# chenxy99/Scanpaths

Hardware: AMD Instinct MI355X
Metric: images/sec/GPU (AiR train step, bs=32, 320x512) at 1/2/4/8 MI355X (higher is better)
Workload: dtype f32; 1 GPU; AiR supervised train step (fwd+loss+bwd+clip+Adam), resnet50, T=16, 320x512, per-GPU batch 32; global_batch=32, parallelism=dp1

## Files before the change

include/scanpaths_amd.h:

```cpp
#ifndef SCANPATHS_AMD_H
#define SCANPATHS_AMD_H
#include <stdint.h>

#ifdef __cplusplus
extern "C" {
#endif

#define SP_OK 0
#define SP_EINVAL (-1)
#define SP_ENULL (-2)

#define SP_ABI_VERSION 4
int sp_abi_version(void);

int sp_set_tuning(const char* name, int value);
int sp_timing_build(void);

typedef struct sp_conv_desc {
    int N_img, Hi, Wi, Kc, ldx;
    int Ho, Wo, Nout, ldc;
    int KH, KW, stride, pad, dil;
    int mode, ldw;
    float alpha;
    int beta, relu;
    int nbatch;
    int64_t strideX, strideW, strideC;
    int ksplit;
    void* workspace;
    int w_scale_rows;
    const int* row_last;
    int row_step;
} sp_conv_desc;

int sp_conv_igemm(const sp_conv_desc* d, const float* X, const float* W, const float* bias, float* out, void* stream);

int sp_split3_bf16(const float* x, int64_t n, void* out, void* stream);
int sp_split3_bf16_wT(const float* w, int Co, int taps, int Ci, void* out, void* stream);
int sp_conv_igemm_bf16x3(const sp_conv_desc* d, const void* Xsplit, const void* Wsplit, const float* bias, float* out,
                         void* stream);

typedef struct sp_wgrad_desc {
    int N_img, Hi, Wi, Ci, ldx;
    int Ho, Wo, Co, ldy;
    int KH, KW, stride, pad, dil;
    int ldo;
    int beta;
    float alpha;
    int nbatch;
    int64_t strideX, strideY, strideO;
    int x_scale_vec, y_scale_vec;
    const int* row_last;
    int row_step;
} sp_wgrad_desc;

int64_t sp_conv_wgrad_workspace(const sp_wgrad_desc* d);
int sp_conv_wgrad(const sp_wgrad_desc* d, const float* X, const float* dY, float* dW, void* workspace, void* stream);

int64_t sp_conv_wgrad_bf16x3_workspace(const sp_wgrad_desc* d);
int sp_conv_wgrad_bf16x3(const sp_wgrad_desc* d, const void* Xsplit, const void* dYsplit, float* dW, void* workspace,
                         void* stream);

int sp_split2_f16(const float* x, int64_t n, void* out, float* scale_amax,
                  int have_amax ,
                  void* stream);
int sp_split2_f16_wT(const float* w, int Co, int taps, int Ci, void* out, float* scale_amax, void* stream);
int sp_split2_f16_rows(const float* w, int64_t rows, int64_t K, int Kc, const float* absorb, void* out, float* row_scale, void* stream);
int sp_split2_f16_wT_rows(const float* w, int nbatch, int Co, int taps, int Ci, const float* absorb, void* out, float* row_scale, void* stream);
int64_t sp_split2_f16_cols_workspace(int64_t rows, int C);
int sp_split2_f16_cols(const float* x, int64_t rows, int C, void* out, float* col_scale, void* scratch, void* stream);
int sp_conv_igemm_f16x2(const sp_conv_desc* d, const void* Xsplit, const float* x_scale, const void* Wsplit, const float* w_scale,
                        const float* bias, float* out, void* stream);
int64_t sp_conv_wgrad_f16x2_workspace(const sp_wgrad_desc* d);
int sp_conv_wgrad_f16x2(const sp_wgrad_desc* d, const void* Xsplit, const float* x_scale, const void* dYsplit,
                        const float* y_scale, float* dW, void* workspace, void* stream);
int64_t sp_conv_wgrad_f16x2_multi_workspace(const sp_wgrad_desc* d, int nseg);
int sp_conv_wgrad_f16x2_multi(const sp_wgrad_desc* d, int nseg, const void* const* Xsplits, const float* const* x_scales,
                              const void* const* dYsplits, const float* const* y_scales, float* dW, void* workspace,
                              const int* row_last, const int* seg_steps, void* stream);
int64_t sp_conv_stats_tiles(const sp_conv_desc* d);
int sp_conv_igemm_f16x2_stats(const sp_conv_desc* d, const void* Xsplit, const float* x_scale, const void* Wsplit,
                              const float* w_scale, float* out, double* st_partial, float* st_mm, void* stream);
int sp_conv_igemm_f16x1(const sp_conv_desc* d, const void* Xsplit, const float* x_scale, const void* Wsplit, const float* w_scale,
                        const float* bias, float* out, void* stream);
int sp_conv_wgrad_f16x1(const sp_wgrad_desc* d, const void* Xsplit, const float* x_scale, const void* dYsplit,
                        const float* y_scale, float* dW, void* workspace, void* stream);
int sp_gateconv_lstm_f16x2(const sp_conv_desc* d, const void* Hsplit, const float* h_scale, const void* Wsplit, const float* w_scale,
                           const float* xg, const float* c_prev, const float* spcol, const float* wc, int P, int KP, float* gates,
                           float* c_out, float* h_out, unsigned* h_amax,
                           void* hout_planes ,
                           float* hout_scale , float hout_bound ,
                           void* stream);
int sp_rank1_grads_applies(int B, int P, int N3, int KP, int ldy);
int64_t sp_rank1_grads_workspace(int B, int P, int N3, int KP);
int sp_rank1_grads_f16x2(const void* dpre_planes, const float* dpre_scale, int ldy, const void* wcT_planes, const float* wcT_row_scale,
                         const float* spcol, int B, int P, int N3, int KP, float* dsp, float* dwc, void* workspace, const int* row_last,
                         int row_step, void* stream);


int64_t sp_colsum_workspace(int64_t M, int C);
int sp_colsum(const float* x, int64_t M, int C, int ld, float* out, int beta, void* workspace, void* stream);
int sp_rowsum(const float* x, int64_t M, int C, float scale, float* out, void* stream);
int sp_rowsum_bwd(const float* dout, int64_t M, int C, float scale, float* dx, void* stream);

int64_t sp_bn_workspace(int64_t M, int C);
int sp_bn_stats(const float* x, int64_t M, int C, float eps, float momentum, float* mean, float* invstd,
                float* running_mean, float* running_var, void* workspace, void* stream);
int sp_bn_eval_stats(const float* running_mean, const float* running_var, int C, float eps, float* mean,
                     float* invstd, void* stream);
int sp_bn_apply(const float* x, const float* mean, const float* invstd, const float* gamma, const float* beta,
                const float* residual, int relu, int64_t M, int C, float* y,
                unsigned* y_amax , void* stream);
int sp_bn_backward(const float* dy, const float* x, const float* y, const float* mean, const float* invstd,
                   const float* gamma, int relu, int training, int64_t M, int C, float* dx, float* dres,
                   float* dgamma, float* dbeta, void* workspace,
                   unsigned* dx_amax , void* stream);

int64_t sp_bn_split_workspace(int64_t M, int C);
int64_t sp_bn_mask_words(int64_t M, int C);
int sp_bn_fwd_split(const float* x, int64_t M, int C, float eps, float momentum, const float* gamma, const float* beta,
                    const float* residual, const unsigned* res_amax, int relu, float* mean, float* invstd, float* running_mean,
                    float* running_var, float* ext, float* y, void* planes, float* y_scale, unsigned* bound,
                    unsigned long long* mask, void* workspace,
                    const double* pre_partial ,
                    const float* pre_mm , int pre_G, void* stream);
int sp_bn_bwd_split(const float* dy, const float* x, const unsigned long long* mask, const float* mean, const float* invstd,
                    const float* gamma, const float* ext, int64_t M, int C, float* dx, float* dres, void* planes, float* dx_scale,
                    unsigned* bound, float* dgamma, float* dbeta, void* workspace, void* stream);

int sp_maxpool3s2_fwd(const float* x, int N, int H, int W, int C, float* y, unsigned char* argmax , int Ho, int Wo,
                      void* stream);
int sp_maxpool3s2_bwd(const float* dy, const unsigned char* argmax, int N, int H, int W, int C, float* dx, int Ho, int Wo, void* stream);
int sp_nchw_to_nhwc_pad(const float* x, int N, int C, int H, int W, int Cp, float* y, void* stream);
int sp_pad_lastdim(const float* x, int64_t rows, int Cin, int Cout, float* y, void* stream);
int sp_sum_n(const float* const* inputs, int count, int64_t n, float* out, unsigned* out_amax, const int* row_last, const int* steps,
             int nsamples, void* stream);
int sp_sum_n_mixed(const float* const* inputs, const void* const* planes, const float* const* scales, int count, int64_t n, float* out,
                   unsigned* out_amax, const int* row_last, const int* steps, int nsamples, void* stream);
int sp_relu_bwd(const float* dy, const float* y, int64_t n, float* dx, void* stream);
int sp_add(const float* a, const float* b, float* out, int64_t n, void* stream);

int sp_lstm_pointwise_fwd(const float* xg, const float* hg, const float* c_prev, int64_t rows, int C, float* gates,
                          float* c_out, float* h_out, void* stream);
int sp_lstm_rank1_fwd(const float* xg, const float* hg, const float* c_prev, const float* spcol, const float* wc, int B, int P,
                      int C, int KP, float* gates, float* c_out, float* h_out,
                      unsigned* h_amax , void* stream);
int64_t sp_rank1_dwc_workspace(int B, int P, int N3, int KP);
int sp_rank1_dwc(const float* dpre, const float* spcol, int B, int P, int ld, int N3, int KP, void* workspace, float* dwc,
                 void* stream);
int64_t sp_sempool_workspace(int S, int B, int P, int C);
int sp_sempool_fwd(const float* a, const float* vf, int S, int B, int P, int C, float alpha, void* workspace, float* out, int sbc,
                   void* stream);
int sp_sempool_bwd(const float* dout, const float* out, const float* a, const float* vf, int S, int B, int P, int C, float alpha,
                   float* da, float* dvf, const int* row_last, int row_step, int sbc, void* stream);
int sp_lstm_pointwise_bwd(const float* dh, const float* dc, const float* gates, const float* c_prev, const float* c_out,
                          int64_t rows, int C, float* dpre, float* dc_prev, unsigned* dpre_amax, unsigned* dcp_amax,
                          const unsigned* dh_amax, const unsigned* dc_amax, float c_bound, float cprev_bound, void* planes,
                          float* dpre_scale, const int* row_last, int row_step, int rows_per_sample, void* stream);

int sp_im2col3x3_1ch(const float* maps, int S, int R, int H, int W, int ldk, float* col, void* stream);
int sp_col2im3x3_1ch(const float* dcol, int S, int R, int H, int W, int ldk, float* dmaps, void* stream);

int sp_listatt_fwd(const float* L, const float* u, int T, int R, int D, float* mem, float* alpha, void* stream);
int sp_listatt_bwd(const float* dmem, const float* L, const float* u, const float* alpha, int T, int R, int D, float* dL,
                   float* du_partial, void* stream);

int sp_mulrelu_fwd(const float* a, const float* b, int64_t n, int64_t nb, float* out, void* stream);
int sp_mulrelu_bwd(const float* dout, const float* a, const float* b, const float* out, int64_t n, int64_t nb, float* da,
                   float* db_partial, void* stream);

int sp_select_rows(const float* a, const float* b, const unsigned char* sel, int64_t rows, int64_t len, float* out,
                   void* stream);
int sp_select_rows_bwd(const float* dout, const unsigned char* sel, int64_t rows, int64_t len, float* da, float* db,
                       void* stream);

int sp_head_finish_fwd(const float* Z, int B, int Hm, int Wm, int ldz, int nheads, int HC, const float* cb,
                       int cb_per_sample , const float* w2, const float* b2, int softmax, float* logits, float* amap, float* mu,
                       float* sigma2, float* drt,
                       const float* dpre ,
                       int zc , int parts, void* stream);
int sp_head_finish_bwd(const float* dlogits, int64_t dlogits_ld, const float* damap , const float* dmu,
                       const float* dsigma2, const float* logits, const float* amap, const float* sigma2, const float* drt, int B, int Hm,
                       int Wm, int ldz, int nheads, int HC, const float* w2, int softmax, float* dZ, float* dcb_partial,
                       float* dw2_partial, float* db2_partial,
                       float* ddpre ,
                       int zc, int parts, int* live, void* stream);

int sp_head_num_classes(int Hm, int Wm);
int sp_head_compose11_fwd(const float* G, const float* cb, int nheads, int HC, int C, int Hm, int Wm, float* W11,
                          float* cbsum, void* stream);
int sp_head_compose11_bwd(const float* dW11, const float* dcbsum, int nheads, int HC, int C, int Hm, int Wm, float* dG,
                          float* dcb, void* stream);
int sp_sal_gather_fwd(const float* T, int B, int Hm, int Wm, int ldt, int nsel, const int* hmap, float* Z2, void* stream);
int sp_sal_gather_bwd(const float* dZ2, int B, int Hm, int Wm, int ldt, int nsel, int nsrc, const int* hmap, float* dT,
                      const int* row_last, int row_step, void* stream);
int sp_drt_direct_fwd(const float* h, const float* W11, const float* cbsum, const int* hmap, int B, int Hm, int Wm, int C,
                      int nsel, float* Dpre, void* stream);
int sp_drt_direct_bwd_data(const float* dDpre, const float* W11, const int* hmap, int B, int Hm, int Wm, int C, int nsel,
                           int accumulate, float* dh, const int* live, const int* row_last, int row_step, int rowB, void* stream);
int64_t sp_drt_direct_bwd_weight_workspace(int B, int Hm, int Wm, int C, int nsel);
int sp_drt_direct_bwd_weight(const float* dDpre, const float* h, const int* hmap, int B, int Hm, int Wm, int C, int nsel, int nheads,
                             void* workspace, float* dW11, float* dcbsum, const int* live, const int* row_last, int row_step, int rowB,
                             void* stream);

int sp_gemm_skinny_applies(int M, int N, int K, int lda, int ldb, int ldc, int layout);
int64_t sp_gemm_skinny_workspace(int M, int N, int K, int layout);
int sp_gemm_skinny(const float* A, const float* B, const float* bias, float* C, int M, int N, int K, int lda, int ldb, int ldc, int layout,
                   float alpha, int relu, void* workspace, void* stream);

int64_t sp_scanpath_loss_workspace(int B, int T);
int sp_scanpath_loss(const float* z, const float* gt, const float* amask, const float* mu, const float* sigma2,
// ... 105 lines not shown
```

scanpaths_amd/config.py:

```python
from __future__ import annotations

import os
import sys

DEFAULTS = {
    "split_scheme": "f16x2", "use_split": True, "library": "product", "always_reset_amax": False,
    "fused_amax": True, "grad_merge": True, "bn_split": True, "bn_skip_dx": True, "bn_skip_z": True, "lstm_bwd_split": True,
    "rank1_dsp_split": True, "rank1_dwc_split": True, "lstm_skip_dpre": True, "fuse_gate_lstm": True, "lstm_h_planes": True,
    "defer_wgrad": True, "channel_scales": True, "hw2_single": True, "row_sparsity": True, "direct_grad": True, "skinny_gemm": True, "async_dgrad": True,
    "drt_batched": True, "rank1_fused": True,
}
_off = lambda v: v != "0"
_ENV = {
    "SP_SPLIT_SCHEME": ("split_scheme", str), "SP_NO_SPLIT": ("use_split", lambda v: not v), "SP_LIBRARY": ("library", str),
    "SP_ALWAYS_RESET_AMAX": ("always_reset_amax", bool), "SP_NO_AMAX_HINT": ("fused_amax", lambda v: not v),
    "SP_GRAD_MERGE": ("grad_merge", _off), "SP_BN_SPLIT": ("bn_split", _off), "SP_BN_SKIP_DX": ("bn_skip_dx", _off),
    "SP_BN_SKIP_Z": ("bn_skip_z", _off), "SP_LSTM_BWD_SPLIT": ("lstm_bwd_split", _off), "SP_RANK1_DSP_SPLIT": ("rank1_dsp_split", _off),
    "SP_RANK1_DWC_SPLIT": ("rank1_dwc_split", _off), "SP_LSTM_SKIP_DPRE": ("lstm_skip_dpre", _off), "SP_FUSE_LSTM": ("fuse_gate_lstm", _off),
    "SP_LSTM_H_PLANES": ("lstm_h_planes", _off), "SP_DEFER_WGRAD": ("defer_wgrad", _off), "SP_CHANNEL_SCALES": ("channel_scales", _off),
    "SP_HW2_SINGLE": ("hw2_single", _off), "SP_ROW_SPARSITY": ("row_sparsity", _off), "SP_DIRECT_GRAD": ("direct_grad", _off), "SP_SKINNY_GEMM": ("skinny_gemm", _off),
    "SP_ASYNC_DGRAD": ("async_dgrad", _off), "SP_DRT_BATCHED": ("drt_batched", _off), "SP_RANK1_FUSED": ("rank1_fused", _off),
}
TIMING_KNOBS = {"SP_H2_DBG": b"h2_dbg", "SP_HW_DBG": b"hw_dbg", "SP_B3_DBG": b"b3_dbg", "SP_HW_SPLITS": b"hw_splits", "SP_H2_HALO": b"h2_halo",
                "SP_ROW_ORDER": b"row_order", "SP_HW_CAP": b"hw_cap"}

settings = dict(DEFAULTS)
_announced = set()


def env_tuning_allowed() -> bool:
    return os.environ.get("SP_ALLOW_ENV_TUNING") == "1"


def _loud(msg: str) -> None:
    if msg not in _announced:
        _announced.add(msg)
        print(f"scanpaths_amd.config: {msg}", file=sys.stderr, flush=True)


def _check(name, value):
    if name not in DEFAULTS:
        raise KeyError(f"scanpaths_amd.config: unknown switch {name!r} (known: {sorted(DEFAULTS)})")
    if name == "split_scheme" and value not in ("f16x2", "bf16x3", "f16x1"):
        raise ValueError(f"split_scheme must be f16x2, bf16x3 or f16x1, got {value!r}")
    if name == "library" and value not in ("product", "timing"):
        raise ValueError(f"library must be product or timing, got {value!r}")
    if name == "split_scheme" and value == "f16x1":
        _loud("THROUGHPUT MODE selected (split_scheme=f16x1): GEMM operands rounded to ONE fp16 plane -- about 100x off the 1e-4 parity "
              "bar; results are NOT comparable with the fp32 reference")
    if name == "library" and value == "timing":
        _loud("TIMING LIBRARY selected (libscanpaths_amd_timing.so): contains wrong-result timing modes; for tools/ only")


def _load_env():
    present = [k for k in list(_ENV) + list(TIMING_KNOBS) if os.environ.get(k) not in (None, "")]
    if not present:
        return
    if not env_tuning_allowed():
        _loud(f"IGNORING {', '.join(present)}: environment tuning needs SP_ALLOW_ENV_TUNING=1 (set switches in code with "
              "scanpaths_amd.config.set)")
        return
    for k in present:
        if k in _ENV:
            name, parse = _ENV[k]
            v = parse(os.environ[k])
            _check(name, v)
            settings[name] = v


def set(**kw) -> None:
    for k, v in kw.items():
        _check(k, v)
        if k == "library" and "scanpaths_amd.hip" in sys.modules and sys.modules["scanpaths_amd.hip"]._lib is not None \
                and v != settings["library"]:
            raise RuntimeError("scanpaths_amd.config: the library is already loaded; choose it before the first launch")
        settings[k] = v
    f = sys.modules.get("scanpaths_amd.functional")
    if f is not None:
        f._apply_config()
    h = sys.modules.get("scanpaths_amd.hip")
    if h is not None and "library" in kw:
        h._apply_config()


def honour_env_for_tools() -> None:
    os.environ["SP_ALLOW_ENV_TUNING"] = "1"
    _load_env()
    for name in ("scanpaths_amd.functional", "scanpaths_amd.hip"):
        m = sys.modules.get(name)
        if m is not None:
            if name.endswith("hip") and m._lib is not None and (settings["library"] == "timing") != m.TIMING_LIB:
                raise RuntimeError("scanpaths_amd.config: the library is already loaded; call honour_env_for_tools() before the first launch")
            m._apply_config()


def non_default() -> dict:
    return {k: v for k, v in settings.items() if v != DEFAULTS[k]}


_load_env()
# ... 1 lines not shown
```

scanpaths_amd/csrc/bn_pool.hip:

```cpp
#include "common.h"
#include <algorithm>

namespace {

__device__ __forceinline__ int64_t sp_cdiv_dev(int64_t a, int64_t b) { return (a + b - 1) / b; }

constexpr int CB = 64;
constexpr int RL = 16;
constexpr int MAX_G = 256;

inline int pick_G_wide(int64_t M, int C) {
    const int64_t colblocks = sp_cdiv(C, 256);
    int64_t g = sp_cdiv(1024, colblocks);
    g = std::min<int64_t>(g, sp_cdiv(M, 4 * 8));
    g = std::min<int64_t>(g, 1024);
    return (int)std::max<int64_t>(g, 1);
}

inline int pick_G(int64_t M, int C) {
    const int64_t colblocks = sp_cdiv(C, CB);
    int64_t g = sp_cdiv(2048, colblocks);
    g = std::min<int64_t>(g, sp_cdiv(M, RL * 8));
    g = std::min<int64_t>(g, MAX_G);
    return (int)std::max<int64_t>(g, 1);
// ... 852 lines not shown
extern "C" int sp_bn_apply(const float* x, const float* mean, const float* invstd, const float* gamma, const float* beta,
                           const float* residual, int relu, int64_t M, int C, float* y, unsigned* y_amax, void* stream) {
    if (!x || !mean || !invstd || !gamma || !beta || !y) return SP_ENULL;
    if (C % 4) return SP_EINVAL;
    const int64_t n4 = M * C / 4;
    SP_RESET_AMAX(y_amax, stream);
    hipLaunchKernelGGL(bn_apply_kernel, dim3(ew_blocks(n4)), dim3(256), 0, (hipStream_t)stream, x, mean, invstd, gamma,
                       beta, residual, relu, n4, C, y, y_amax);
    SP_LAUNCH_CHECK();
    return SP_OK;
}

extern "C" int sp_bn_backward(const float* dy, const float* x, const float* y, const float* mean, const float* invstd,
                              const float* gamma, int relu, int training, int64_t M, int C, float* dx, float* dres,
                              float* dgamma, float* dbeta, void* workspace, unsigned* dx_amax, void* stream) {
    if (!dy || !x || !mean || !invstd || !gamma || !dx || !dgamma || !dbeta || !workspace) return SP_ENULL;
    if (relu && !y) return SP_ENULL;
    if (C % 4 || M <= 0) return SP_EINVAL;
    hipStream_t s = (hipStream_t)stream;
    const int G = pick_G(M, C);
    double* partial = (double*)workspace;
    float* coef = (float*)(partial + (int64_t)G * 2 * C);
    hipLaunchKernelGGL(bn_bwd_partial, dim3((unsigned)sp_cdiv(C, CB), G), dim3(256), 0, s, dy, x, y, mean, invstd, relu, M,
                       C, G, partial);
    SP_LAUNCH_CHECK();
    hipLaunchKernelGGL(bn_bwd_final, dim3((unsigned)sp_cdiv(C, FIN_C)), dim3(FIN_C * FIN_L), 0, s, partial, M, C, G, dgamma, dbeta,
                       coef);
    SP_LAUNCH_CHECK();
    const int64_t n4 = M * C / 4;
    SP_RESET_AMAX(dx_amax, s);
    hipLaunchKernelGGL(bn_bwd_apply, dim3(ew_blocks(n4)), dim3(256), 0, s, dy, x, y, mean, invstd, gamma, coef, relu,
                       training, n4, C, dx, dres, dx_amax);
    SP_LAUNCH_CHECK();
    return SP_OK;
}

extern "C" int64_t sp_bn_split_workspace(int64_t M, int C) {
    const int64_t G = std::max(pick_G(M, C), pick_G_wide(M, C));
    return G * 2 * C * (int64_t)sizeof(double) + G * 2 * C * (int64_t)sizeof(float) + 2 * (int64_t)C * (int64_t)sizeof(float);
}

extern "C" int64_t sp_bn_mask_words(int64_t M, int C) { return sp_cdiv(M * C / 4, 64) * 4; }

extern "C" int sp_bn_fwd_split(const float* x, int64_t M, int C, float eps, float momentum, const float* gamma, const float* beta,
                               const float* residual, const unsigned* res_amax, int relu, float* mean, float* invstd,
                               float* running_mean, float* running_var, float* ext, float* y, void* planes, float* y_scale,
                               unsigned* bound, unsigned long long* mask, void* workspace, const double* pre_partial,
                               const float* pre_mm, int pre_G, void* stream) {
    if (!x || !gamma || !beta || !mean || !invstd || !ext || !y_scale || !bound || !workspace) return SP_ENULL;
    if ((residual && !res_amax) || (relu && !mask) || (!y && !planes)) return SP_ENULL;
    if (C % 4 || (planes && C % 16) || M <= 0 || ((uintptr_t)planes & 15)) return SP_EINVAL;
    hipStream_t s = (hipStream_t)stream;
    int G = pick_G(M, C);
    const double* partial = (double*)workspace;
    const float* mm = (float*)((double*)workspace + (int64_t)G * 2 * C);
    SP_RESET_AMAX(bound, s);
    if (pre_partial) {
        if (!pre_mm || pre_G < 1) return SP_EINVAL;
        partial = pre_partial;
        mm = pre_mm;
        G = pre_G;
    } else {
        hipLaunchKernelGGL(bn_stats_mm_partial, dim3((unsigned)sp_cdiv(C, CB), G), dim3(256), 0, s, x, M, C, G, (double*)workspace,
                           (float*)((double*)workspace + (int64_t)G * 2 * C));
        SP_LAUNCH_CHECK();
    }
    if (G > 256)
        hipLaunchKernelGGL((bn_stats_mm_final<8, 32>), dim3((unsigned)sp_cdiv(C, 8)), dim3(256), 0, s, partial, mm, M, C, G, eps,
                           momentum, gamma, beta, relu, mean, invstd, running_mean, running_var, ext, bound);
    else
        hipLaunchKernelGGL((bn_stats_mm_final<FIN_C, FIN_L>), dim3((unsigned)sp_cdiv(C, FIN_C)), dim3(256), 0, s, partial, mm, M, C,
                           G, eps, momentum, gamma, beta, relu, mean, invstd, running_mean, running_var, ext, bound);
    SP_LAUNCH_CHECK();
    const int64_t n4 = M * C / 4;
    hipLaunchKernelGGL(bn_apply_split_kernel, dim3(ew_blocks(n4)), dim3(256), 0, s, x, mean, invstd, gamma, beta, residual, bound,
                       residual ? res_amax : nullptr, relu, n4, C, y, (uint16_t*)planes, y_scale, relu ? mask : nullptr);
    SP_LAUNCH_CHECK();
    return SP_OK;
}

extern "C" int sp_bn_bwd_split(const float* dy, const float* x, const unsigned long long* mask, const float* mean,
                               const float* invstd, const float* gamma, const float* ext, int64_t M, int C, float* dx,
                               float* dres, void* planes, float* dx_scale, unsigned* bound, float* dgamma, float* dbeta,
                               void* workspace, void* stream) {
    if (!dy || !x || !mean || !invstd || !gamma || !ext || !dx_scale || !bound || !dgamma || !dbeta || !workspace) return SP_ENULL;
    if (!dx && !planes) return SP_ENULL;
    if (C % 4 || (planes && C % 16) || M <= 0 || ((uintptr_t)planes & 15)) return SP_EINVAL;
    hipStream_t s = (hipStream_t)stream;
    const bool wide = C >= 256 && C % 256 == 0;
    const int G = wide ? pick_G_wide(M, C) : pick_G(M, C);
    double* partial = (double*)workspace;
    float* dmax = (float*)(partial + (int64_t)G * 2 * C);
    float* coef = dmax + (int64_t)G * 2 * C;
    SP_RESET_AMAX(bound, s);
    if (wide)
        hipLaunchKernelGGL(bn_bwd_mm_partial<64>, dim3((unsigned)(C / 256), G), dim3(256), 0, s, dy, x, mask, mean, invstd, M, C, G,
                           partial, dmax);
    else
        hipLaunchKernelGGL(bn_bwd_mm_partial<16>, dim3((unsigned)sp_cdiv(C, CB), G), dim3(256), 0, s, dy, x, mask, mean, invstd, M, C,
                           G, partial, dmax);
    SP_LAUNCH_CHECK();
    if (G > 256)
        hipLaunchKernelGGL((bn_bwd_mm_final<8, 32>), dim3((unsigned)sp_cdiv(C, 8)), dim3(256), 0, s, partial, dmax, M, C, G, gamma,
                           mean, invstd, ext, dgamma, dbeta, coef, bound);
    else
        hipLaunchKernelGGL((bn_bwd_mm_final<FIN_C, FIN_L>), dim3((unsigned)sp_cdiv(C, FIN_C)), dim3(256), 0, s, partial, dmax, M, C,
                           G, gamma, mean, invstd, ext, dgamma, dbeta, coef, bound);
    SP_LAUNCH_CHECK();
    const int64_t n4 = M * C / 4;
    hipLaunchKernelGGL(bn_bwd_apply_split_kernel, dim3(ew_blocks(n4)), dim3(256), 0, s, dy, x, mask, mean, invstd, gamma, coef,
                       bound, n4, C, dx, dres, (uint16_t*)planes, dx_scale);
    SP_LAUNCH_CHECK();
    return SP_OK;
}

extern "C" int64_t sp_colsum_workspace(int64_t M, int C) { return (int64_t)pick_G(M, C) * C * (int64_t)sizeof(double); }

extern "C" int sp_colsum(const float* x, int64_t M, int C, int ld, float* out, int beta, void* workspace, void* stream) {
    if (!x || !out || !workspace) return SP_ENULL;
    if (C % 4 || ld % 4 || M <= 0) return SP_EINVAL;
    hipStream_t s = (hipStream_t)stream;
    if (M <= COLSUM_SMALL_M && ((uintptr_t)x & 15) == 0 && ((uintptr_t)out & 15) == 0) {
        hipLaunchKernelGGL(colsum_small_kernel, dim3((unsigned)sp_cdiv(C, 256)), dim3(64), 0, s, x, (int)M, C, ld, out, beta);
        SP_LAUNCH_CHECK();
        return SP_OK;
    }
    const int G = pick_G(M, C);
    hipLaunchKernelGGL(colsum_partial, dim3((unsigned)sp_cdiv(C, CB), G), dim3(256), 0, s, x, M, C, ld, G, (double*)workspace);
    SP_LAUNCH_CHECK();
    hipLaunchKernelGGL(colsum_final, dim3((unsigned)sp_cdiv(C, FIN_C)), dim3(FIN_C * FIN_L), 0, s, (const double*)workspace, C, G, out,
                       beta);
    SP_LAUNCH_CHECK();
    return SP_OK;
}

extern "C" int sp_rowsum(const float* x, int64_t M, int C, float scale, float* out, void* stream) {
    if (!x || !out) return SP_ENULL;
    if (C % 4) return SP_EINVAL;
    const int blocks = (int)std::max<int64_t>(1, std::min<int64_t>(sp_cdiv(M, 4), 4096));
    hipLaunchKernelGGL(rowsum_kernel, dim3(blocks), dim3(256), 0, (hipStream_t)stream, x, M, C, scale, out);
    SP_LAUNCH_CHECK();
    return SP_OK;
}

extern "C" int sp_rowsum_bwd(const float* dout, int64_t M, int C, float scale, float* dx, void* stream) {
    if (!dout || !dx) return SP_ENULL;
    if (C % 4) return SP_EINVAL;
    const int64_t n4 = M * C / 4;
    hipLaunchKernelGGL(rowsum_bwd_kernel, dim3(ew_blocks(n4)), dim3(256), 0, (hipStream_t)stream, dout, n4, C, scale, dx);
    SP_LAUNCH_CHECK();
    return SP_OK;
}

extern "C" int sp_maxpool3s2_fwd(const float* x, int N, int H, int W, int C, float* y, unsigned char* argmax, int Ho, int Wo,
                                 void* stream) {
    if (!x || !y) return SP_ENULL;
    if (C % 4) return SP_EINVAL;
    const int64_t total = (int64_t)N * Ho * Wo * (C / 4);
    hipLaunchKernelGGL(maxpool_fwd_kernel, dim3(ew_blocks(total)), dim3(256), 0, (hipStream_t)stream, x, N, H, W, C, y, Ho, Wo,
                       argmax);
    SP_LAUNCH_CHECK();
    return SP_OK;
}

extern "C" int sp_maxpool3s2_bwd(const float* dy, const unsigned char* argmax, int N, int H, int W, int C, float* dx, int Ho,
                                 int Wo, void* stream) {
    if (!dy || !argmax || !dx) return SP_ENULL;
    if (C % 4) return SP_EINVAL;
    const int64_t total = (int64_t)N * H * W * (C / 4);
    hipLaunchKernelGGL(maxpool_bwd_idx_kernel, dim3(ew_blocks(total) * 4), dim3(256), 0, (hipStream_t)stream, dy, argmax, N, H, W,
                       C, dx, Ho, Wo);
    SP_LAUNCH_CHECK();
    return SP_OK;
}

extern "C" int sp_nchw_to_nhwc_pad(const float* x, int N, int C, int H, int W, int Cp, float* y, void* stream) {
    if (!x || !y) return SP_ENULL;
    if (Cp < C) return SP_EINVAL;
    const int64_t total = (int64_t)N * H * W * Cp;
    hipLaunchKernelGGL(nchw_to_nhwc_pad_kernel, dim3(ew_blocks(total)), dim3(256), 0, (hipStream_t)stream, x, N, C, H, W, Cp, y);
    SP_LAUNCH_CHECK();
    return SP_OK;
}
// ... 76 lines not shown
```

scanpaths_amd/csrc/conv_f16x2.hip:

```cpp
#include "common.h"
#include <algorithm>
#include <cstdlib>

typedef _Float16 f16x8 __attribute__((ext_vector_type(8)));

namespace {

#define SP_GLDS16(src, dst)                                                                                      \
    __builtin_amdgcn_global_load_lds((const __attribute__((address_space(1))) void*)(src),                       \
                                     (__attribute__((address_space(3))) void*)(dst), 16, 0, 0)

constexpr int HBM = 256, HBN = 128, HBK = 32;
constexpr int HA_BYTES = HBM * 128;
constexpr int HB_BYTES = HBN * 128;
constexpr int HSTAGE = HA_BYTES + HB_BYTES;
constexpr int HNSTAGE = 3;
constexpr int HCHUNK_KT = 8;
constexpr int HALO_W = 64, HALO_ROWSLOTS = HALO_W + 2, HALO_NSLOT = 6 * HALO_ROWSLOTS;
constexpr int HALO_PIECES = (HALO_NSLOT + 7) / 8;
constexpr int HALO_A_BYTES = HALO_PIECES * 1024;
constexpr int HALO_LDS = 2 * HALO_A_BYTES + 3 * HB_BYTES;

struct H2Args {
    const uint16_t* X;
    const uint16_t* W;
    const float* bias;
    float* C;
    const float* sx;
    const float* sw;
    int sw_rows;
    int64_t M;
    int Hi, Wi, Kc;
    int ldx;
    int Ho, Wo, Nout, ldc;
    int KH, KW, stride, pad, dil;
    int64_t ldwb;
    int64_t w_bstride;
    int rows_per_batch;
    int ncblk, nkt, tiles_n;
    float alpha;
    int beta, relu;
    uint32_t x_bytes, w_bytes;
    const float* l_xg;
    const float* l_cprev;
    const float* l_spcol;
    const float* l_wc;
    float* l_gates;
    float* l_c;
    float* l_h;
    unsigned* l_hamax;
    uint16_t* l_hplanes;
    float* l_hscale;
    float l_hbound;
    int lC, lP, lKP;
    int l_probe;
    double* st_partial;
    float* st_mm;
    const int* row_last;
    int row_step;
    int row_nimg;
};

__device__ __forceinline__ float h2_sigmoid(float x) { return sp_sigmoid(x); }
__device__ __forceinline__ int halo_swz(int slot) { return ((slot >> 1) & 3) << 1; }

template <int MODE, int NPROD, bool CBM, bool LSTM = false, bool HALO = false, int DBG = 0>
__global__ __launch_bounds__(512, 2) void h2_kernel(H2Args p) {
    static_assert(!LSTM || MODE == 0, "the LSTM epilogue belongs to the forward build");
    static_assert(!HALO || (CBM && NPROD == 3 && DBG == 0), "the halo build extends the channel-block-major schedule only");
    extern __shared__ __attribute__((aligned(16))) unsigned char smem[];
    constexpr bool LSTM_T = LSTM;
    const int t = threadIdx.x;
    const int lane = t & 63;
    const int wave = __builtin_amdgcn_readfirstlane(t >> 6);
    const int wm = wave >> 1, wn = wave & 1;

#ifdef SP_TIMING_VARIANTS
    const int probe = p.l_probe;
    if ((probe >> 8) && blockIdx.x < 256) {
        const int G = (probe >> 8) & 15, step_us = 2 * ((probe >> 12) & 31);
        const long long wait = (long long)((blockIdx.x >> 3) % G) * step_us * 100;
        const long long t0 = __builtin_amdgcn_s_memrealtime();
        while ((long long)__builtin_amdgcn_s_memrealtime() - t0 < wait) __builtin_amdgcn_s_sleep(32);
    }
#else
    constexpr int probe = 0;
#endif
    const float sx_dev = p.sx[0], sw_dev = p.sw_rows ? 1.f : p.sw[0];
    int tn, tmi;
    bool mapped = false;
    if constexpr (MODE == 1 && !LSTM) {
        if (p.row_nimg > 0) {
            const int mine = lane < p.row_nimg ? p.row_last[lane] : -1;
            const uint64_t lm = __ballot(lane < p.row_nimg && mine >= p.row_step);
            const uint64_t all = p.row_nimg == 64 ? ~0ull : ((1ull << p.row_nimg) - 1ull);
            const int tps = (p.Ho * p.Wo) / HBM;
            const int nlive = __popcll(lm);
            const int nl = nlive * tps * p.tiles_n;
            const int bid = blockIdx.x;
            uint64_t mask;
            int tml;
            if (bid < nl) {
                supertile_map(xcd_remap(bid, nl), nlive * tps, p.tiles_n, tml, tn, CBM);
                mask = lm;
            } else {
                tn = (bid - nl) % p.tiles_n;
                tml = (bid - nl) / p.tiles_n;
                mask = all & ~lm;
            }
            for (int k = tml / tps; k > 0; --k) mask &= mask - 1ull;
            tmi = (__ffsll((unsigned long long)mask) - 1) * tps + tml % tps;
            mapped = true;
        }
    }
    if (!mapped) supertile_map(xcd_remap(blockIdx.x, gridDim.x), gridDim.x / p.tiles_n, p.tiles_n, tmi, tn, CBM);
    const int64_t m0 = (int64_t)tmi * HBM;
    const int n0 = LSTM ? tn * 32 : tn * HBN;
    if constexpr (!LSTM) {
        if (p.row_last != nullptr) {
            const int howo = MODE == 1 ? p.Ho * p.Wo : p.rows_per_batch;
            const int img = (int)(m0 / howo);
            if (howo % HBM == 0 && m0 < p.M && p.row_last[img] < p.row_step) {
                if (!p.beta) {
                    for (int i = t; i < HBM * (HBN / 4); i += 512) {
                        const int row = i / (HBN / 4), n = n0 + (i % (HBN / 4)) * 4;
                        const int64_t m = m0 + row;
                        if (m >= p.M) continue;
                        float* dst = p.C + m * p.ldc + n;
                        if ((p.ldc & 3) == 0 && n + 3 < p.Nout && (reinterpret_cast<uintptr_t>(p.C) & 15) == 0) {
                            *reinterpret_cast<float4*>(dst) = make_float4(0.f, 0.f, 0.f, 0.f);
                        } else {
                            for (int e = 0; e < 4; ++e)
                                if (n + e < p.Nout) dst[e] = 0.f;
                        }
                    }
                }
                return;
            }
        }
    }
    const int HoWo = p.Ho * p.Wo;

    int a_c8[4], a_py[4], a_px[4], a_boff[4];
    bool a_rowok[4];
// ... 562 lines not shown
            if (t == 0) {
                p.l_hscale[0] = hsc;
                p.l_hscale[1] = p.l_hbound;
            }
        }
        if (p.l_hamax) {
#pragma unroll
            for (int off = 32; off >= 1; off >>= 1) hmx = fmaxf(hmx, __shfl_xor(hmx, off));
            if (lane == 0 && hmx > 0.f) atomicMax(p.l_hamax, __float_as_uint(hmx));
        }
        return;
    }
    {
        const bool stats = MODE == 0 && p.st_partial != nullptr;
        const bool wide = (p.ldc & 3) == 0 && (p.Nout & 3) == 0 && (reinterpret_cast<uintptr_t>(p.C) & 15) == 0;
        float* stg = reinterpret_cast<float*>(smem) + wave * (64 * 68);
        const bool full_m = m0 + HBM <= p.M;
        double cs[4], cq[4];
        float cmn[4], cmx[4];
#pragma unroll
        for (int j = 0; j < 4; ++j) {
            const int n = n0 + wn * 64 + j * 16 + l16;
            const bool n_ok = n < p.Nout;
            const float bv = (n_ok && p.bias) ? p.bias[n] : 0.f;
            const float iswn = (p.sw_rows && n_ok) ? 1.f / ((!LSTM && !HALO) ? pre_sw[j] : p.sw[swrow0 + n]) : isw;
            cs[j] = 0.0;
            cq[j] = 0.0;
            cmn[j] = INFINITY;
            cmx[j] = -INFINITY;
            if (wide && full_m) {
                if (n_ok) {
                    if (stats) {
#pragma unroll
                        for (int i = 0; i < 4; ++i)
#pragma unroll
                            for (int r = 0; r < 4; ++r) {
                                const float v = p.alpha * (((tot4[i][j][r] + acc4[i][j][r]) * isx) * iswn) + bv;
                                stg[(i * 16 + 4 * g4 + r) * 68 + j * 16 + l16] = v;
                                cs[j] += (double)v;
                                cq[j] += (double)v * (double)v;
                                cmn[j] = fminf(cmn[j], v);
                                cmx[j] = fmaxf(cmx[j], v);
                            }
                    } else {
#pragma unroll
                        for (int i = 0; i < 4; ++i)
#pragma unroll
                            for (int r = 0; r < 4; ++r)
                                stg[(i * 16 + 4 * g4 + r) * 68 + j * 16 + l16] = p.alpha * (((tot4[i][j][r] + acc4[i][j][r]) * isx) * iswn) + bv;
                    }
                }
                continue;
            }
#pragma unroll
            for (int i = 0; i < 4; ++i)
#pragma unroll
                for (int r = 0; r < 4; ++r) {
                    const int row = i * 16 + 4 * g4 + r;
                    const int64_t m = m0 + wm * 64 + row;
                    float v = p.alpha * (((tot4[i][j][r] + acc4[i][j][r]) * isx) * iswn) + bv;
                    if (wide) {
                        stg[row * 68 + j * 16 + l16] = v;
                    } else if (n_ok && m < p.M) {
                        float* dst = p.C + m * p.ldc + n;
                        if (p.beta) v += *dst;
                        if (p.relu) v = fmaxf(v, 0.f);
                        *dst = v;
                    }
                    if (stats && n_ok && m < p.M) {
                        cs[j] += (double)v;
                        cq[j] += (double)v * (double)v;
                        cmn[j] = fminf(cmn[j], v);
                        cmx[j] = fmaxf(cmx[j], v);
                    }
                }
        }
        if (wide) {
            asm volatile("s_waitcnt lgkmcnt(0)" ::: "memory");
            const int cq4 = lane & 15, rsub = lane >> 4;
            const int n = n0 + wn * 64 + 4 * cq4;
            if (full_m && n0 + HBN <= p.Nout && !p.relu) {
                float* dst0 = p.C + (m0 + wm * 64 + rsub) * p.ldc + n;
                const float* src0 = stg + rsub * 68 + 4 * cq4;
                if (!p.beta) {
#pragma unroll
                    for (int ps = 0; ps < 16; ++ps)
                        *reinterpret_cast<float4*>(dst0 + (int64_t)(ps * 4) * p.ldc) = *reinterpret_cast<const float4*>(src0 + ps * 4 * 68);
                } else {
                    float4 o[16];
#pragma unroll
                    for (int ps = 0; ps < 16; ++ps) o[ps] = *reinterpret_cast<const float4*>(dst0 + (int64_t)(ps * 4) * p.ldc);
#pragma unroll
                    for (int ps = 0; ps < 16; ++ps) {
                        float4 v = *reinterpret_cast<const float4*>(src0 + ps * 4 * 68);
                        v.x += o[ps].x; v.y += o[ps].y; v.z += o[ps].z; v.w += o[ps].w;
                        *reinterpret_cast<float4*>(dst0 + (int64_t)(ps * 4) * p.ldc) = v;
                    }
                }
            } else
#pragma unroll
            for (int ps = 0; ps < 16; ++ps) {
                const int row = ps * 4 + rsub;
                const int64_t m = m0 + wm * 64 + row;
                if (m < p.M && n < p.Nout) {
                    float4 v = *reinterpret_cast<const float4*>(stg + row * 68 + 4 * cq4);
                    float4* dst = reinterpret_cast<float4*>(p.C + m * p.ldc + n);
                    if (p.beta) {
                        const float4 o = *dst;
                        v.x += o.x; v.y += o.y; v.z += o.z; v.w += o.w;
                    }
                    if (p.relu) {
                        v.x = fmaxf(v.x, 0.f); v.y = fmaxf(v.y, 0.f); v.z = fmaxf(v.z, 0.f); v.w = fmaxf(v.w, 0.f);
                    }
                    *dst = v;
                }
            }
        }
        if (stats) {
            asm volatile("s_waitcnt lgkmcnt(0)" ::: "memory");
            __builtin_amdgcn_s_barrier();
            double* sh_s = reinterpret_cast<double*>(smem);
            float* sh_m = reinterpret_cast<float*>(smem + 4 * HBN * 2 * sizeof(double));
#pragma unroll
            for (int j = 0; j < 4; ++j) {
#pragma unroll
                for (int off = 16; off <= 32; off <<= 1) {
                    cs[j] += __shfl_xor(cs[j], off);
                    cq[j] += __shfl_xor(cq[j], off);
                    cmn[j] = fminf(cmn[j], __shfl_xor(cmn[j], off));
                    cmx[j] = fmaxf(cmx[j], __shfl_xor(cmx[j], off));
                }
                if (g4 == 0) {
                    const int col = wn * 64 + j * 16 + l16;
                    sh_s[(wm * HBN + col) * 2 + 0] = cs[j];
                    sh_s[(wm * HBN + col) * 2 + 1] = cq[j];
                    sh_m[(wm * HBN + col) * 2 + 0] = cmn[j];
                    sh_m[(wm * HBN + col) * 2 + 1] = cmx[j];
                }
            }
            asm volatile("s_waitcnt lgkmcnt(0)" ::: "memory");
            __builtin_amdgcn_s_barrier();
            if (t < HBN && n0 + t < p.Nout) {
                double a = 0.0, b = 0.0;
                float mn = INFINITY, mx = -INFINITY;
#pragma unroll
                for (int w = 0; w < 4; ++w) {
                    a += sh_s[(w * HBN + t) * 2 + 0];
                    b += sh_s[(w * HBN + t) * 2 + 1];
                    mn = fminf(mn, sh_m[(w * HBN + t) * 2 + 0]);
                    mx = fmaxf(mx, sh_m[(w * HBN + t) * 2 + 1]);
                }
                const int64_t g = m0 / HBM;
                p.st_partial[(g * 2 + 0) * p.Nout + n0 + t] = a;
                p.st_partial[(g * 2 + 1) * p.Nout + n0 + t] = b;
                p.st_mm[(g * 2 + 0) * p.Nout + n0 + t] = mn;
                p.st_mm[(g * 2 + 1) * p.Nout + n0 + t] = mx;
            }
        }
    }
}

struct HWArgs {
    const uint16_t* X;
    const uint16_t* dY;
    float* out;
    const float* sx;
    const float* sy;
// ... 916 lines not shown
extern "C" int sp_split2_f16(const float* x, int64_t n, void* out, float* scale_amax, int have_amax, void* stream) {
    if (!x || !out || !scale_amax) return SP_ENULL;
    if (n % 16) return SP_EINVAL;
    hipStream_t s = (hipStream_t)stream;
    unsigned* amax = reinterpret_cast<unsigned*>(scale_amax + 1);
    if (!have_amax) {
        const int rc = launch_amax(x, n, amax, s);
        if (rc != SP_OK) return rc;
    }
    const int64_t n4 = n / 4;
    const int blocks = (int)std::max<int64_t>(1, std::min<int64_t>(sp_cdiv(n4, 256), 4096));
    hipLaunchKernelGGL(split2_kernel, dim3(blocks), dim3(256), 0, s, x, n4, amax, (uint16_t*)out, scale_amax);
    SP_LAUNCH_CHECK();
    return SP_OK;
}

extern "C" int sp_split2_f16_wT(const float* w, int Co, int taps, int Ci, void* out, float* scale_amax, void* stream) {
    if (!w || !out || !scale_amax) return SP_ENULL;
    if (((int64_t)taps * Co) % 16) return SP_EINVAL;
    hipStream_t s = (hipStream_t)stream;
    unsigned* amax = reinterpret_cast<unsigned*>(scale_amax + 1);
    const int64_t total = (int64_t)Co * taps * Ci;
    const int rc = launch_amax(w, total, amax, s);
    if (rc != SP_OK) return rc;
    const int blocks = (int)std::max<int64_t>(1, std::min<int64_t>(sp_cdiv(total, 256), 4096));
    hipLaunchKernelGGL(split2_wT_kernel, dim3(blocks), dim3(256), 0, s, w, Co, taps, Ci, amax, (uint16_t*)out, scale_amax);
    SP_LAUNCH_CHECK();
    return SP_OK;
}


extern "C" int sp_split2_f16_rows(const float* w, int64_t rows, int64_t K, int Kc, const float* absorb, void* out, float* row_scale,
                                  void* stream) {
    if (!w || !out || !row_scale) return SP_ENULL;
    if (rows < 1 || K < 16 || K % 16 || (absorb && (Kc < 4 || Kc % 4 || K % Kc))) return SP_EINVAL;
    if (rows > 0x7fffffff || (((uintptr_t)w | (uintptr_t)absorb) & 15)) return SP_EINVAL;
    hipLaunchKernelGGL(split2_rows_kernel, dim3((unsigned)rows), dim3(256), 0, (hipStream_t)stream, w, K, Kc, absorb, (uint16_t*)out,
                       row_scale, rows);
    SP_LAUNCH_CHECK();
    return SP_OK;
}

extern "C" int sp_split2_f16_wT_rows(const float* w, int nbatch, int Co, int taps, int Ci, const float* absorb, void* out,
                                     float* row_scale, void* stream) {
    if (!w || !out || !row_scale) return SP_ENULL;
    if (nbatch < 1 || nbatch > 65535 || ((int64_t)taps * Co) % 16 || Ci % 4 || Ci < 4 || ((uintptr_t)w & 15)) return SP_EINVAL;
    hipLaunchKernelGGL(split2_wT_rows_kernel, dim3(Ci / 4, nbatch), dim3(256), 0, (hipStream_t)stream, w, Co, taps, Ci, absorb, (uint16_t*)out,
                       row_scale);
    SP_LAUNCH_CHECK();
    return SP_OK;
}

static int colamax_blocks(int64_t rows, int C_) {
    const int C4 = C_ / 4, cg_per = std::min(C4, 256), rpb = 256 / cg_per;
    return (int)std::max<int64_t>(1, std::min<int64_t>(sp_cdiv(rows, (int64_t)rpb * 4), COLAMAX_MAXBLK));
}
extern "C" int64_t sp_split2_f16_cols_workspace(int64_t rows, int C_) {
    if (rows < 1 || C_ < 16 || C_ % 16) return 0;
    return (int64_t)colamax_blocks(rows, C_) * C_ * (int64_t)sizeof(float);
}
extern "C" int sp_split2_f16_cols(const float* x, int64_t rows, int C_, void* out, float* col_scale, void* scratch, void* stream) {
    if (!x || !out || !col_scale || !scratch) return SP_ENULL;
    if (rows < 1 || C_ < 16 || C_ % 16 || (((uintptr_t)x | (uintptr_t)col_scale | (uintptr_t)scratch) & 15)) return SP_EINVAL;
    hipStream_t s = (hipStream_t)stream;
    const int nblk = colamax_blocks(rows, C_);
    hipLaunchKernelGGL(colamax_partial_kernel, dim3(nblk), dim3(256), 0, s, x, rows, C_, (float*)scratch);
    SP_LAUNCH_CHECK();
    hipLaunchKernelGGL(colamax_final_kernel, dim3((unsigned)sp_cdiv(C_, 32)), dim3(256), 0, s, (const float*)scratch, nblk, C_, col_scale);
    SP_LAUNCH_CHECK();
    const int64_t n4 = rows * (C_ / 4);
    const int blocks2 = (int)std::max<int64_t>(1, std::min<int64_t>(sp_cdiv(n4, 256), 4096));
    hipLaunchKernelGGL(split2_cols_kernel, dim3(blocks2), dim3(256), 0, s, x, n4, C_, (const float*)col_scale, (uint16_t*)out);
    SP_LAUNCH_CHECK();
    return SP_OK;
}

static bool halo_applies(const sp_conv_desc* d) {
    return d->KH == 3 && d->KW == 3 && d->stride == 1 && d->dil == 1 && d->pad == 1 && d->Wo == HALO_W && d->Wi == HALO_W &&
           d->Hi == d->Ho && (d->Ho * d->Wo) % HBM == 0 && d->Kc % 32 == 0;
}

static int conv_igemm_f16(const sp_conv_desc* d, const void* Xs, const float* x_scale, const void* Ws, const float* w_scale,
                          const float* bias, float* out, void* stream, int nprod, double* st_partial = nullptr,
                          float* st_mm = nullptr) {
    if (!d || !Xs || !Ws || !x_scale || !w_scale || !out) return SP_ENULL;
    if (d->mode != 0 && d->mode != 1) return SP_EINVAL;
    if (d->Kc % 32 || d->ldx < d->Kc || d->ldx % 16) return SP_EINVAL;
    if (((uintptr_t)Xs | (uintptr_t)Ws) & 15) return SP_EINVAL;
    if (d->nbatch < 1 || d->stride < 1 || d->dil < 1) return SP_EINVAL;
    const int64_t rows_b = (int64_t)d->N_img * d->Ho * d->Wo;
    if (d->nbatch > 1) {
        if (d->mode != 0 || d->KH * d->KW != 1 || d->stride != 1 || d->pad != 0 || rows_b % HBM || rows_b >= (1LL << 31)) return SP_EINVAL;
        if (d->strideX != rows_b * d->ldx || d->strideC != rows_b * d->ldc || d->strideW != (int64_t)d->Nout * d->Kc) return SP_EINVAL;
        if (st_partial || nprod != 3) return SP_EINVAL;
    }
    H2Args a{};
    a.X = (const uint16_t*)Xs; a.W = (const uint16_t*)Ws; a.bias = bias; a.C = out;
    a.sx = x_scale; a.sw = w_scale; a.sw_rows = d->w_scale_rows ? 1 : 0;
    a.row_last = ((d->mode == 1 && d->nbatch == 1) || (d->mode == 0 && d->nbatch > 1)) ? d->row_last : nullptr; a.row_step = d->row_step;
    a.row_nimg = (a.row_last && d->mode == 1 && d->nbatch == 1 && d->N_img <= 64 && ((int64_t)d->Ho * d->Wo) % HBM == 0 &&
                  sp_tuning_get(SP_TUNE_ROW_ORDER, 1) == 1) ? d->N_img : 0;
    a.M = rows_b * d->nbatch;
    a.Hi = d->Hi; a.Wi = d->Wi; a.Kc = d->Kc; a.ldx = d->ldx;
    a.Ho = d->Ho; a.Wo = d->Wo; a.Nout = d->Nout; a.ldc = d->ldc;
    a.KH = d->KH; a.KW = d->KW; a.stride = d->stride; a.pad = d->pad; a.dil = d->dil;
    a.w_bstride = d->nbatch > 1 ? 4 * d->strideW : 0;
    a.rows_per_batch = (int)rows_b;
    a.ldwb = 4 * (int64_t)d->KH * d->KW * d->Kc;
    a.ncblk = d->Kc / 32;
    a.nkt = d->KH * d->KW * a.ncblk;
    a.tiles_n = (int)sp_cdiv(d->Nout, HBN);
    a.alpha = d->alpha; a.beta = d->beta; a.relu = d->relu;
    const int64_t xb = 4LL * d->nbatch * d->N_img * d->Hi * d->Wi * d->ldx, wb = 4LL * d->nbatch * d->Nout * d->KH * d->KW * d->Kc;
    if (xb + 64 >= (1LL << 32) || wb + 64 >= (1LL << 32)) return SP_EINVAL;
    a.x_bytes = (uint32_t)xb; a.w_bytes = (uint32_t)wb;
    if (a.M <= 0 || a.M >= (1LL << 31) || a.Nout <= 0) return SP_EINVAL;
    hipStream_t st = (hipStream_t)stream;
    const bool f = d->mode == 0;
    const bool cbm_ok = d->KH * d->KW > 1 && d->KH * d->KW <= 32 && (f || d->stride == 1);
    if (st_partial) {
        if (!f || !st_mm || nprod != 3 || d->beta || d->relu || bias) return SP_EINVAL;
        a.st_partial = st_partial; a.st_mm = st_mm;
        return cbm_ok ? launch_h2<0, 3, true>(a, st) : launch_h2<0, 3, false>(a, st);
    }
#ifdef SP_TIMING_VARIANTS
    if (sp_tuning_get(SP_TUNE_H2_DBG, 0) >= 256) a.l_probe = sp_tuning_get(SP_TUNE_H2_DBG, 0) & ~255;
    switch (sp_tuning_get(SP_TUNE_H2_DBG, 0)) {
        case 6: return f ? launch_h2<0, 3, false, false, false, 1>(a, st) : launch_h2<1, 3, false, false, false, 1>(a, st);
        case 7: return f ? launch_h2<0, 3, false, false, false, 2>(a, st) : launch_h2<1, 3, false, false, false, 2>(a, st);
        case 8: return f ? launch_h2<0, 3, false, false, false, 3>(a, st) : launch_h2<1, 3, false, false, false, 3>(a, st);
        case 9: return f ? launch_h2<0, 3, false, false, false, 9>(a, st) : launch_h2<1, 3, false, false, false, 9>(a, st);
        default: break;
    }
#endif
    if (nprod == 1)
        return f ? launch_h2<0, 1, false>(a, st) : launch_h2<1, 1, false>(a, st);
    if (cbm_ok && halo_applies(d) && sp_tuning_get(SP_TUNE_H2_HALO, 1) == 1)
        return f ? launch_h2<0, 3, true, false, true>(a, st) : launch_h2<1, 3, true, false, true>(a, st);
    if (cbm_ok) return f ? launch_h2<0, 3, true>(a, st) : launch_h2<1, 3, true>(a, st);
    return f ? launch_h2<0, 3, false>(a, st) : launch_h2<1, 3, false>(a, st);
}

extern "C" int sp_conv_igemm_f16x2(const sp_conv_desc* d, const void* Xs, const float* x_scale, const void* Ws,
                                   const float* w_scale, const float* bias, float* out, void* stream) {
    return conv_igemm_f16(d, Xs, x_scale, Ws, w_scale, bias, out, stream, 3);
}

extern "C" int64_t sp_conv_stats_tiles(const sp_conv_desc* d) {
    if (!d) return 0;
    return sp_cdiv((int64_t)d->N_img * d->Ho * d->Wo, HBM);
}
extern "C" int sp_conv_igemm_f16x2_stats(const sp_conv_desc* d, const void* Xs, const float* x_scale, const void* Ws,
                                         const float* w_scale, float* out, double* st_partial, float* st_mm, void* stream) {
    if (!st_partial || !st_mm) return SP_ENULL;
    return conv_igemm_f16(d, Xs, x_scale, Ws, w_scale, nullptr, out, stream, 3, st_partial, st_mm);
}

extern "C" int sp_conv_igemm_f16x1(const sp_conv_desc* d, const void* Xs, const float* x_scale, const void* Ws,
                                   const float* w_scale, const float* bias, float* out, void* stream) {
    return conv_igemm_f16(d, Xs, x_scale, Ws, w_scale, bias, out, stream, 1);
}

extern "C" int sp_gateconv_lstm_f16x2(const sp_conv_desc* d, const void* Hs, const float* h_scale, const void* Ws,
                                      const float* w_scale, const float* xg, const float* c_prev, const float* spcol,
                                      const float* wc, int P, int KP, float* gates, float* c_out, float* h_out, unsigned* h_amax,
                                      void* hout_planes, float* hout_scale, float hout_bound, void* stream) {
    if (!d || !Hs || !Ws || !h_scale || !w_scale || !xg || !spcol || !wc || !gates || !c_out || !h_out) return SP_ENULL;
    if (d->mode != 0 || d->Kc % 32 || d->ldx != d->Kc || d->nbatch != 1 || d->stride != 1 || d->dil < 1) return SP_EINVAL;
    if (d->Nout != 4 * d->Kc || d->Ho != d->Hi || d->Wo != d->Wi || d->KH * d->KW < 2 || d->KH * d->KW > 32) return SP_EINVAL;
    if (P != d->Ho * d->Wo || P % HBM || KP < 1 || KP > 32) return SP_EINVAL;
    if (((uintptr_t)Hs | (uintptr_t)Ws) & 15) return SP_EINVAL;
    if (((uintptr_t)xg | (uintptr_t)c_prev | (uintptr_t)gates | (uintptr_t)c_out | (uintptr_t)h_out) & 15) return SP_EINVAL;
    if (d->w_scale_rows && ((uintptr_t)w_scale & 15)) return SP_EINVAL;
    H2Args a{};
    a.X = (const uint16_t*)Hs; a.W = (const uint16_t*)Ws; a.bias = nullptr; a.C = nullptr;
    a.sx = h_scale; a.sw = w_scale; a.sw_rows = d->w_scale_rows ? 1 : 0;
    a.M = (int64_t)d->N_img * P;
    a.Hi = d->Hi; a.Wi = d->Wi; a.Kc = d->Kc; a.ldx = d->Kc;
    a.Ho = d->Ho; a.Wo = d->Wo; a.Nout = d->Nout; a.ldc = d->Nout;
    a.KH = d->KH; a.KW = d->KW; a.stride = 1; a.pad = d->pad; a.dil = d->dil;
    a.ldwb = 4 * (int64_t)d->KH * d->KW * d->Kc;
    a.ncblk = d->Kc / 32;
    a.nkt = d->KH * d->KW * a.ncblk;
    a.tiles_n = d->Kc / 32;
    a.alpha = 1.f; a.beta = 0; a.relu = 0;
    const int64_t xb = 4LL * a.M * d->Kc, wb = 4LL * d->Nout * d->KH * d->KW * d->Kc;
    if (xb + 64 >= (1LL << 32) || wb + 64 >= (1LL << 32) || a.M <= 0) return SP_EINVAL;
    a.x_bytes = (uint32_t)xb; a.w_bytes = (uint32_t)wb;
    a.l_xg = xg; a.l_cprev = c_prev; a.l_spcol = spcol; a.l_wc = wc;
    if (hout_planes && (!hout_scale || !(hout_bound > 0.f) || ((uintptr_t)hout_planes & 15))) return SP_EINVAL;
    a.l_gates = gates; a.l_c = c_out; a.l_h = h_out; a.l_hamax = h_amax;
    a.l_hplanes = (uint16_t*)hout_planes; a.l_hscale = hout_scale; a.l_hbound = hout_bound;
    a.lC = d->Kc; a.lP = P; a.lKP = KP;
    a.l_probe = sp_tuning_get(SP_TUNE_H2_DBG, 0);
    hipStream_t st = (hipStream_t)stream;
    SP_RESET_AMAX(h_amax, st);
    if (halo_applies(d) && sp_tuning_get(SP_TUNE_H2_HALO, 1) == 1) return launch_h2<0, 3, true, true, true>(a, st);
    return launch_h2<0, 3, true, true, false>(a, st);
}

extern "C" int64_t sp_conv_wgrad_f16x2_workspace(const sp_wgrad_desc* d) {
    if (!d) return 0;
    if (d->nbatch > 1) return 0;
    const int sp = hw_splits(d);
    return sp <= 1 ? 0 : (int64_t)sp * d->Co * d->ldo * (int64_t)sizeof(float);
}

static int launch_hw_reduce(const HWScales& sc, const float* slab, float* dW, int Co, int Ntot, int ldo, int splits, int64_t slab_stride,
                            float alpha, int beta, hipStream_t s) {
    const int64_t total = (int64_t)Co * Ntot;
    if (Ntot % 4 == 0 && ldo % 4 == 0 && slab_stride % 4 == 0 && sc.Ci % 4 == 0 && (((uintptr_t)slab | (uintptr_t)dW) & 15) == 0) {
        const int blocks = (int)std::min<int64_t>(sp_cdiv(total / 4, 256), 4096);
        hipLaunchKernelGGL(hw_reduce4_kernel, dim3(blocks), dim3(256), 0, s, slab, dW, Co, Ntot / 4, ldo / 4, splits, slab_stride / 4, alpha, sc, beta);
    } else {
        const int blocks = (int)std::min<int64_t>(sp_cdiv(total, 256), 4096);
        hipLaunchKernelGGL(hw_reduce_kernel, dim3(blocks), dim3(256), 0, s, slab, dW, Co, Ntot, ldo, splits, slab_stride, alpha, sc, beta);
    }
    SP_LAUNCH_CHECK();
    return SP_OK;
}

static int conv_wgrad_f16(const sp_wgrad_desc* d, const void* Xsplit, const float* x_scale, const void* dYsplit,
                          const float* y_scale, float* dW, void* workspace, void* stream, int nprod) {
    if (!d || !Xsplit || !dYsplit || !x_scale || !y_scale || !dW) return SP_ENULL;
    if (d->Ci % 16 || d->Co % 16 || d->ldx != d->Ci || d->ldy < d->Co || d->ldy % 16 || d->nbatch < 1) return SP_EINVAL;
    if (((uintptr_t)Xsplit | (uintptr_t)dYsplit) & 15) return SP_EINVAL;
    const int64_t rows_b = (int64_t)d->N_img * d->Ho * d->Wo;
    const bool batched = d->nbatch > 1;
    if (batched) {
        if (d->KH * d->KW != 1 || d->stride != 1 || d->pad != 0 || rows_b % 32 || nprod != 3) return SP_EINVAL;
        if (d->strideX != rows_b * d->Ci || d->strideY != rows_b * d->ldy || d->strideO != (int64_t)d->Co * d->ldo) return SP_EINVAL;
    } else if (d->ldo < d->KH * d->KW * d->Ci) {
        return SP_EINVAL;
    }
    HWArgs a;
    a.X = (const uint16_t*)Xsplit; a.dY = (const uint16_t*)dYsplit;
    a.sx = x_scale; a.sy = y_scale;
    a.sx_vec = d->x_scale_vec ? 1 : 0; a.sy_vec = d->y_scale_vec ? 1 : 0;
// ... 128 lines not shown
```

scanpaths_amd/functional.py:

```python
from __future__ import annotations

import ctypes as C
from collections import namedtuple
from typing import Optional

import torch
from torch.autograd import Function

from . import config as _config
from . import hip
from .hip import ConvDesc, WgradDesc, check, ptr


_KSPLIT_MIN_NKT, _KSPLIT_KT = 8, 4


def _timed(key_flops, launch):
    if hip.TIMER is None:
        return launch()
    return hip.TIMER.bracket(*key_flops(), launch)


def _gemm_desc(M, Nout, Kc, *, ldx, ldw, ldc, mode=0, alpha=1.0, beta=0, relu=0, nbatch=1, sX=0, sW=0, sC=0):
    return ConvDesc(N_img=M, Hi=1, Wi=1, Kc=Kc, ldx=ldx, Ho=1, Wo=1, Nout=Nout, ldc=ldc, KH=1, KW=1, stride=1, pad=0, dil=1, mode=mode,
                    ldw=ldw, alpha=float(alpha), beta=int(beta), relu=int(relu), nbatch=nbatch, strideX=sX, strideW=sW, strideC=sC)


def _gemm_wgrad_desc(M, Co, Ci, *, ldx, ldy, ldo, alpha=1.0, nbatch=1, sX=0, sY=0, sO=0):
    return WgradDesc(N_img=M, Hi=1, Wi=1, Ci=Ci, ldx=ldx, Ho=1, Wo=1, Co=Co, ldy=ldy, KH=1, KW=1, stride=1, pad=0, dil=1, ldo=ldo,
                     alpha=float(alpha), nbatch=nbatch, strideX=sX, strideY=sY, strideO=sO)


def _igemm(d: ConvDesc, X, W, bias, out):
    M_, Nout, Kc, mode, taps, nbatch = d.N_img * d.Ho * d.Wo, d.Nout, d.Kc, d.mode, d.KH * d.KW, d.nbatch
    aligned = all(t is None or t.data_ptr() % 16 == 0 for t in (X, W, out, bias))
    if (SKINNY_GEMM and taps == 1 and nbatch == 1 and M_ <= 64 and not d.beta and d.Hi == d.Ho and d.Wi == d.Wo and d.stride == 1
            and d.pad == 0 and aligned and d.ldc % 4 == 0 and hip.lib().sp_gemm_skinny_applies(M_, Nout, Kc, d.ldx, d.ldw, d.ldc, mode)):
        L = hip.lib()
        ws = hip.workspace(L.sp_gemm_skinny_workspace(M_, Nout, Kc, mode), X.device, slot=2)

        def launch_sk():
            check(L.sp_gemm_skinny(ptr(X), ptr(W), ptr(bias), ptr(out), M_, Nout, Kc, d.ldx, d.ldw, d.ldc, mode, d.alpha, d.relu,
                                   ptr(ws), hip.stream()), "sp_gemm_skinny")
        FUSION_COUNTS["skinny_gemm"] += 1
        return _timed(lambda: (("skinny_fwd" if mode == 0 else "skinny_dgrad", M_, Nout, Kc, "1x1", 1), 2.0 * M_ * Nout * Kc), launch_sk)
    if taps == 1 and nbatch == 1:
        tiles = ((M_ + 127) // 128) * ((Nout + 127) // 128)
        nkt = (Kc + 31) // 32
        if tiles <= 64 and nkt >= _KSPLIT_MIN_NKT:
            d.ksplit = max(2, min(nkt // _KSPLIT_KT, 512 // tiles))
            d.workspace = ptr(hip.workspace(d.ksplit * M_ * Nout * 4, X.device, slot=2))

    def launch():
        check(hip.lib().sp_conv_igemm(C.byref(d), ptr(X), ptr(W), ptr(bias), ptr(out), hip.stream()), "sp_conv_igemm")
    _timed(lambda: (("igemm_fwd" if mode == 0 else "igemm_dgrad", M_, Nout, taps * Kc, f"{d.KH}x{d.KW}", nbatch),
                    2.0 * M_ * Nout * taps * Kc * nbatch), launch)


def _wgrad(d: WgradDesc, X, dY, dW):
    L = hip.lib()
    ws = hip.workspace(L.sp_conv_wgrad_workspace(C.byref(d)), X.device, slot=0)
    def launch():
        check(L.sp_conv_wgrad(C.byref(d), ptr(X), ptr(dY), ptr(dW), ptr(ws), hip.stream()), "sp_conv_wgrad")
    _timed(lambda: (("wgrad", d.N_img * d.Ho * d.Wo, d.Co, d.KH * d.KW * d.Ci, f"{d.KH}x{d.KW}", d.nbatch),
                    2.0 * d.N_img * d.Ho * d.Wo * d.Co * d.KH * d.KW * d.Ci * d.nbatch), launch)


def _apply_config():
    g = globals()
    c = _config.settings
    g["FUSED_AMAX"] = bool(c["fused_amax"])
    g["USE_BF16X3"] = bool(c["use_split"])
    g["THROUGHPUT_MODE"] = c["split_scheme"] == "f16x1"
    g["SPLIT_SCHEME"] = "f16x2" if c["split_scheme"] == "f16x1" else c["split_scheme"]
    for name, key in (("GRAD_MERGE", "grad_merge"), ("BN_SPLIT", "bn_split"), ("BN_SKIP_DX", "bn_skip_dx"), ("BN_SKIP_Z", "bn_skip_z"),
                      ("LSTM_BWD_SPLIT", "lstm_bwd_split"), ("RANK1_DSP_SPLIT", "rank1_dsp_split"), ("RANK1_DWC_SPLIT", "rank1_dwc_split"),
                      ("LSTM_SKIP_DPRE", "lstm_skip_dpre"), ("FUSE_GATE_LSTM", "fuse_gate_lstm"), ("LSTM_H_PLANES", "lstm_h_planes"),
                      ("DEFER_WGRAD", "defer_wgrad"), ("CHANNEL_SCALES", "channel_scales"), ("HW2_SINGLE", "hw2_single"),
                      ("ROW_SPARSITY", "row_sparsity"), ("DIRECT_GRAD", "direct_grad"), ("SKINNY_GEMM", "skinny_gemm"), ("ASYNC_DGRAD", "async_dgrad"),
                      ("DRT_BATCHED", "drt_batched"), ("RANK1_FUSED", "rank1_fused")):
        g[name] = bool(c[key])


_apply_config()


FUSION_COUNTS = {"lstm_bwd_split": 0, "bn_bwd_split_operand": 0, "gateconv_lstm": 0, "gateconv_lstm_hplanes": 0,
                 "bn_fwd_split": 0, "bn_fwd_split_operand": 0, "bn_skip_z": 0, "bn_bwd_split": 0, "bn_skip_dx": 0,
                 "conv_bn_stats": 0, "grad_merge": 0, "rank1_dsp_split": 0, "rank1_dwc_split": 0, "lstm_skip_dpre": 0, "wgrad_multi": 0,
                 "row_sparse_bwd": 0, "fan_in_rows": 0, "direct_grad": 0, "output_gate": 0, "skinny_gemm": 0, "async_dgrad": 0,
                 "drt_fwd_batched": 0, "rank1_fused": 0}


def _grad_slot(param):
    if not DIRECT_GRAD or param is None or not getattr(param, "is_leaf", False) or not param.requires_grad:
        return None
    if getattr(param, "_sp_flat", None) is None:
        return None
    if getattr(param, "_backward_hooks", None):
        return None
    try:
        return param, torch.autograd.graph.get_gradient_edge(param).node
    except Exception:
        return None


def _take_grad_view(pn, phys_perm=None):
    if pn is None:
        return None, None
    param, node = pn
    try:
        if not torch._C._will_engine_execute_node(node):
            return None, None
    except RuntimeError:
        return None, None
    slot = param._sp_flat
    g = slot.peek(param)
    if g is None:
        return None, None
    v = g.permute(*phys_perm) if phys_perm is not None else g
    if not v.is_contiguous():
        return None, None
    slot.take()
    FUSION_COUNTS["direct_grad"] += 1
    return slot, v


class RowsCtx:
    __slots__ = ("last", "B")

    def __init__(self, last):
        self.last, self.B = last, int(last.numel())


class DecodeRows:
    __slots__ = ("rc",)

    def __init__(self):
        self.rc = None

    def at(self, t: int) -> "DecodeStep":
        return DecodeStep(t, self)


class DecodeStep(int):
    def __new__(cls, t, rows):
        o = int.__new__(cls, t)
        o.rows = rows
        return o


def rows_ctx(step, nsamples):
    tok = getattr(step, "rows", None)
    if tok is None or not ROW_SPARSITY:
        return None
    rc = tok.rc
    if rc is None or rc.B != nsamples:
        return None
    return rc


class _OutputGate(Function):
    @staticmethod
    def forward(ctx, tok, *outs):
        ctx.tok = tok
        ctx.set_materialize_grads(False)
        return tuple(o.view_as(o) for o in outs)

    @staticmethod
    def backward(ctx, *grads):
        tok = ctx.tok
        tok.rc = None
        live = [g for g in grads if g is not None]
        if ROW_SPARSITY and live:
# ... 122 lines not shown
        n = xc.numel()
        out = torch.empty(2 * n + 32, dtype=torch.float16, device=x.device)
        Cc = xc.shape[-1]
        if channel and CHANNEL_SCALES and hint is None and xc.dim() >= 2 and Cc % 16 == 0 and not THROUGHPUT_MODE:
            cscale = torch.empty(Cc, dtype=torch.float32, device=x.device)
            L = hip.lib()
            ws = hip.workspace(L.sp_split2_f16_cols_workspace(n // Cc, Cc), x.device, slot=1)
            check(L.sp_split2_f16_cols(ptr(xc), n // Cc, Cc, ptr(out), ptr(cscale), ptr(ws), hip.stream()), "sp_split2_f16_cols")
            op = SplitOperand(out, cscale, scheme, "cols")
        else:
            scale = hint if hint is not None else _scale_slot(x.device)
            check(hip.lib().sp_split2_f16(ptr(xc), n, ptr(out), ptr(scale), int(hint is not None), hip.stream()), "sp_split2_f16")
            op = SplitOperand(out, scale, scheme)
    if cache is not None:
        cache[scheme] = op
    return op


def _absorb_of(act: Optional[SplitOperand]) -> Optional[torch.Tensor]:
    return act.scale if (act is not None and act.kind == "cols") else None


def split_w(w2d: torch.Tensor, scheme: str, Kc: Optional[int] = None, absorb: Optional[torch.Tensor] = None) -> SplitOperand:
    if scheme == "bf16x3":
        return SplitOperand(split3(w2d), None, scheme)
    w2d = w2d.contiguous()
    K = w2d.shape[-1]
    rows = w2d.numel() // K
    out = torch.empty(2 * w2d.numel() + 32, dtype=torch.float16, device=w2d.device)
    rscale = torch.empty(rows, dtype=torch.float32, device=w2d.device)
    check(hip.lib().sp_split2_f16_rows(ptr(w2d), rows, K, Kc if Kc is not None else K, ptr(absorb), ptr(out), ptr(rscale), hip.stream()),
          "sp_split2_f16_rows")
    return SplitOperand(out, rscale, scheme, "rows", absorb)


def split_op_wT(wp: torch.Tensor, scheme: Optional[str] = None, absorb: Optional[torch.Tensor] = None) -> SplitOperand:
    Co, KH, KW, Ci = wp.shape
    scheme = scheme or _scheme_for(Co)
    if scheme == "bf16x3":
        return SplitOperand(split3_wT(wp), None, scheme)
    out = torch.empty(2 * wp.numel() + 32, dtype=torch.float16, device=wp.device)
    if Ci % 4 == 0:
        rscale = torch.empty(Ci, dtype=torch.float32, device=wp.device)
        check(hip.lib().sp_split2_f16_wT_rows(ptr(wp), 1, Co, KH * KW, Ci, ptr(absorb), ptr(out), ptr(rscale), hip.stream()),
              "sp_split2_f16_wT_rows")
        return SplitOperand(out, rscale, scheme, "rows", absorb)
    assert absorb is None
    scale = _scale_slot(wp.device)
    check(hip.lib().sp_split2_f16_wT(ptr(wp), Co, KH * KW, Ci, ptr(out), ptr(scale), hip.stream()), "sp_split2_f16_wT")
    return SplitOperand(out, scale, scheme)


def _weight_operand(wp, act: SplitOperand, wcache, transposed=False) -> SplitOperand:
    absorb = _absorb_of(act)
    key = ("wT" if transposed else "w", act.scheme)
    if absorb is None and wcache is not None and key in wcache:
        return wcache[key]
    if transposed:
        op = split_op_wT(wp, act.scheme, absorb)
    else:
        Co, KH, KW, Ci = wp.shape
        op = split_w(wp.reshape(Co, KH * KW * Ci), act.scheme, Ci, absorb)
    if absorb is None and wcache is not None:
        wcache[key] = op
    return op


COST_M_SCALE = 1.0


def _b3_pays(M, N, K, Kc, nbatch=1, a_elems=None, free_a=False):
    if not USE_BF16X3 or nbatch != 1 or Kc % 16 or N < 64:
        return False
    f16 = _scheme_for(Kc) == "f16x2"
    Mc = M * COST_M_SCALE
    flops = 2.0 * Mc * N * K
    split_bytes = (12.0 if f16 else 10.0) * ((0 if free_a else Mc * Kc) + N * K)
    bpe = 4.0 if f16 else 6.0
    if bpe * (a_elems if a_elems is not None else 4.0 * M * Kc) + 64 >= 2 ** 32 or bpe * N * K + 64 >= 2 ** 32:
        return False
    return flops * (1 / 1.1e14 - 1 / (4.0e14 if f16 else 2.5e14)) > split_bytes / 4e12 and flops > (1e9 if free_a else 2e9)


def _igemm_b3(d: ConvDesc, Xs, Ws, bias, out, stats=None, rows=None):
    assert Xs.scheme == Ws.scheme, (Xs.scheme, Ws.scheme)
    f16 = Xs.scheme == "f16x2"
    xscale = Xs.scale
    mode = d.mode
    if f16 and rows is not None and mode == 1:
        d.row_last, d.row_step = rows[0].last.data_ptr(), int(rows[1])
    if f16:
        d.w_scale_rows = int(Ws.kind == "rows")
        if Xs.kind == "cols":
            if Ws.absorbed is not Xs.scale:
                raise RuntimeError("scanpaths_amd: a per-channel-scaled operand met a weight operand that did not absorb its scales")
            xscale = _one(out.device)
        elif Ws.absorbed is not None:
            raise RuntimeError("scanpaths_amd: a weight operand that absorbed per-channel scales met another activation operand")

    def launch():
        if stats is not None:
            check(hip.lib().sp_conv_igemm_f16x2_stats(C.byref(d), ptr(Xs.buf), ptr(xscale), ptr(Ws.buf), ptr(Ws.scale), ptr(out),
                                                      ptr(stats[0]), ptr(stats[1]), hip.stream()), "sp_conv_igemm_f16x2_stats")
        elif f16:
            fn = hip.lib().sp_conv_igemm_f16x1 if THROUGHPUT_MODE else hip.lib().sp_conv_igemm_f16x2
            check(fn(C.byref(d), ptr(Xs.buf), ptr(xscale), ptr(Ws.buf), ptr(Ws.scale), ptr(bias), ptr(out), hip.stream()),
                  "sp_conv_igemm_f16x2")
        else:
            check(hip.lib().sp_conv_igemm_bf16x3(C.byref(d), ptr(Xs.buf), ptr(Ws.buf), ptr(bias), ptr(out), hip.stream()),
                  "sp_conv_igemm_bf16x3")

    def key_flops():
        M = d.N_img * d.Ho * d.Wo
        K = d.KH * d.KW * d.Kc
        pre = ("h1" if THROUGHPUT_MODE else "h2") if f16 else "b3"
        sparse = f16 and rows is not None and mode == 1
        return (pre + ("_fwd" if mode == 0 else "_dgrad") + ("_rows" if sparse else ""), M, d.Nout, K, f"{d.KH}x{d.KW}", 1), 2.0 * M * d.Nout * K
    _timed(key_flops, launch)


def _wgrad_scheme(Ci, Co) -> str:
    return "f16x2" if _scheme_for(Ci) == "f16x2" and _scheme_for(Co) == "f16x2" else "bf16x3"


def _w3_pays(M, Co, K, Ci, nbatch=1, free_splits=False):
    f16 = _wgrad_scheme(Ci, Co) == "f16x2"
    if not USE_BF16X3 or nbatch != 1 or Co % 16 or Co < 64 or (Ci % 128 and not f16):
        return False
    flops = 2.0 * M * COST_M_SCALE * Co * K
    split_bytes = 0.0 if free_splits else (12.0 if f16 else 10.0) * M * COST_M_SCALE * (Ci + Co)
    if 6.0 * M * max(Ci, Co) * 4 >= 2 ** 32:
        return False
    return flops * (1 / 1.0e14 - 1 / (3.2e14 if f16 else 1.6e14)) > split_bytes / 4e12 and flops > 2e9


HW2_SINGLE_MIN_FLOPS = 9e10


def _wgrad_b3(d: WgradDesc, Xs, dYs, dW):
    assert Xs.scheme == dYs.scheme, (Xs.scheme, dYs.scheme)
    L = hip.lib()
    f16 = Xs.scheme == "f16x2"
    if f16:
        d.x_scale_vec, d.y_scale_vec = int(Xs.kind == "cols"), int(dYs.kind == "cols")
    M, Co, K = d.N_img * d.Ho * d.Wo, d.Co, d.KH * d.KW * d.Ci
    big = L.sp_conv_wgrad_f16x2_multi_workspace(C.byref(d), 1) if (f16 and HW2_SINGLE and not THROUGHPUT_MODE
                                                                   and 2.0 * M * COST_M_SCALE * Co * K >= HW2_SINGLE_MIN_FLOPS) else 0
    ws = hip.workspace(big if big > 0 else (L.sp_conv_wgrad_f16x2_workspace if f16 else L.sp_conv_wgrad_bf16x3_workspace)(C.byref(d)),
                       dW.device, slot=0)

    def launch():
        if big > 0:
            FUSION_COUNTS["wgrad_multi"] += 1
            one = lambda t: (C.c_void_p * 1)(t.data_ptr())
            check(L.sp_conv_wgrad_f16x2_multi(C.byref(d), 1, one(Xs.buf), one(Xs.scale), one(dYs.buf), one(dYs.scale), ptr(dW), ptr(ws),
                                              None, None, hip.stream()), "sp_conv_wgrad_f16x2_multi")
        elif f16:
            fn = L.sp_conv_wgrad_f16x1 if THROUGHPUT_MODE else L.sp_conv_wgrad_f16x2
            check(fn(C.byref(d), ptr(Xs.buf), ptr(Xs.scale), ptr(dYs.buf), ptr(dYs.scale), ptr(dW), ptr(ws), hip.stream()),
                  "sp_conv_wgrad_f16x2")
        else:
            check(L.sp_conv_wgrad_bf16x3(C.byref(d), ptr(Xs.buf), ptr(dYs.buf), ptr(dW), ptr(ws), hip.stream()),
                  "sp_conv_wgrad_bf16x3")
    _timed(lambda: (((("h1" if THROUGHPUT_MODE else "h2") if f16 else "b3") + ("_wgrad_multi" if big > 0 else "_wgrad"), M, Co, K, f"{d.KH}x{d.KW}", 1),
                    2.0 * M * Co * K), launch)


class ConvGeom(namedtuple("ConvGeom", "N H W Ci Co KH KW stride pad dil Ho Wo")):
    __slots__ = ()

    @classmethod
    def of(cls, x_shape, Co, KH, KW, stride=1, pad=0, dil=1) -> "ConvGeom":
        N, H, W, Ci = x_shape
        return cls(N, H, W, Ci, Co, KH, KW, stride, pad, dil,
                   (H + 2 * pad - dil * (KH - 1) - 1) // stride + 1, (W + 2 * pad - dil * (KW - 1) - 1) // stride + 1)

    @property
    def M(self) -> int:
        return self.N * self.Ho * self.Wo

    @property
    def K(self) -> int:
        return self.KH * self.KW * self.Ci

    def fwd_desc(self, **kw) -> ConvDesc:
        return ConvDesc(N_img=self.N, Hi=self.H, Wi=self.W, Kc=self.Ci, ldx=self.Ci, Ho=self.Ho, Wo=self.Wo, Nout=self.Co, ldc=self.Co,
                        KH=self.KH, KW=self.KW, stride=self.stride, pad=self.pad, dil=self.dil, mode=0, ldw=self.K, alpha=1.0, nbatch=1, **kw)

    def dgrad_desc(self, split: bool, **kw) -> ConvDesc:
        return ConvDesc(N_img=self.N, Hi=self.Ho, Wi=self.Wo, Kc=self.Co, ldx=self.Co, Ho=self.H, Wo=self.W, Nout=self.Ci, ldc=self.Ci,
                        KH=self.KH, KW=self.KW, stride=self.stride, pad=self.pad, dil=self.dil, mode=1,
                        ldw=self.KH * self.KW * self.Co if split else self.Ci, alpha=1.0, nbatch=1, **kw)

    def wgrad_desc(self, **kw) -> WgradDesc:
        return WgradDesc(N_img=self.N, Hi=self.H, Wi=self.W, Ci=self.Ci, ldx=self.Ci, Ho=self.Ho, Wo=self.Wo, Co=self.Co, ldy=self.Co,
                         KH=self.KH, KW=self.KW, stride=self.stride, pad=self.pad, dil=self.dil, ldo=self.K, alpha=1.0, nbatch=1, **kw)

    def fwd_split(self, free_a=False, a_elems=None) -> bool:
        return _b3_pays(self.M, self.Co, self.K, self.Ci, a_elems=a_elems, free_a=free_a)

    def dgrad_split(self, free_a=False, a_elems=None) -> bool:
        return _b3_pays(self.N * self.H * self.W, self.Ci, self.KH * self.KW * self.Co, self.Co, a_elems=a_elems, free_a=free_a)

    @property
    def wgrad_scheme(self) -> str:
        return _wgrad_scheme(self.Ci, self.Co)

    def wgrad_split(self, free_splits=False) -> Optional[str]:
        return self.wgrad_scheme if _w3_pays(self.M, self.Co, self.K, self.Ci, free_splits=free_splits) else None


def _conv_fwd(g: ConvGeom, x, wp, bias, y, *, relu=False, wcache=None, channel=False, free_a=False, a_elems=None, bn_stats=False):
    d = g.fwd_desc(relu=int(relu))
    if not g.fwd_split(free_a, a_elems):
        _igemm(d, x, wp, bias, y)
        return None, None
    xs = split_op(x, channel=channel)
    wsplit = _weight_operand(wp, xs, wcache)
    stats = None
    if bn_stats and BN_SPLIT and xs.scheme == "f16x2" and not THROUGHPUT_MODE and bias is None and not relu:
        G = hip.lib().sp_conv_stats_tiles(C.byref(d))
        stats = (torch.empty((G, 2, g.Co), dtype=torch.float64, device=x.device),
                 torch.empty((G, 2, g.Co), dtype=torch.float32, device=x.device), G)
    _igemm_b3(d, xs, wsplit, bias, y, stats=stats)
    return xs, stats


def _conv_dgrad(g: ConvGeom, dy, wp, dx, *, dys=None, wcache=None, channel=False, free_a=False, a_elems=None, beta=0, rows=None):
    if not g.dgrad_split(free_a, a_elems):
        _fp32_required(dy, "the fp32 data-gradient GEMM")
        _igemm(g.dgrad_desc(False, beta=beta), dy, wp, None, dx)
        return None
    if dys is None or dys.scheme != _scheme_for(g.Co):
        dys = split_op(dy, channel=channel)
    _igemm_b3(g.dgrad_desc(True, beta=beta), dys, _weight_operand(wp, dys, wcache, transposed=True), None, dx, rows=rows)
    return dys


def _conv_wgrad(g: ConvGeom, x, dy, dwp, *, xs=None, dys=None, channel=False):
    wsch = g.wgrad_scheme
    dy_cached = getattr(dy, "_sp_cache", None)
    if dys is None and dy_cached is not None and wsch in dy_cached:
        dys = dy_cached[wsch]
    if dys is not None and dys.scheme != wsch:
        dys = None
    if g.wgrad_split(free_splits=xs is not None and dys is not None):
        _wgrad_b3(g.wgrad_desc(), xs if xs is not None else split_op(x, wsch, channel=channel),
                  dys if dys is not None else split_op(dy, wsch, channel=channel), dwp)
    else:
        _fp32_required(dy, "the fp32 weight-gradient GEMM")
        _wgrad(g.wgrad_desc(), x, dy, dwp)


def colsum(x2d: torch.Tensor, C_: int, ld: int, M: int) -> torch.Tensor:
    out = torch.empty(C_, dtype=torch.float32, device=x2d.device)
    L = hip.lib()
    ws = hip.workspace(L.sp_colsum_workspace(M, C_), x2d.device, slot=1)
    check(L.sp_colsum(ptr(x2d), M, C_, ld, ptr(out), 0, ptr(ws), hip.stream()), "sp_colsum")
    return out


def _colsum_any(x: torch.Tensor, C_: int) -> torch.Tensor:
    M = x.numel() // C_
    if C_ % 4 == 0:
        return colsum(x, C_, C_, M)
    Cp = (C_ + 3) // 4 * 4
    xp = torch.empty((M, Cp), dtype=torch.float32, device=x.device)
    check(hip.lib().sp_pad_lastdim(ptr(x), M, C_, Cp, ptr(xp), hip.stream()), "sp_pad_lastdim")
    return colsum(xp, Cp, Cp, M)[:C_]


def _add_raw(a: torch.Tensor, b: torch.Tensor) -> torch.Tensor:
    a, b = a.contiguous(), b.contiguous()
    out = torch.empty_like(a)
    check(hip.lib().sp_add(ptr(a), ptr(b), ptr(out), a.numel(), hip.stream()), "sp_add")
    return out


class _Add(Function):
    @staticmethod
    def forward(ctx, a, b):
        return _add_raw(a, b)

    @staticmethod
    def backward(ctx, g):
        return g, g


class _ZeroGradTouch(Function):
    @staticmethod
    def forward(ctx, t, *params):
        ctx.shapes = [(p.shape, p.stride(), p.device) for p in params]
        return t.view_as(t)

    @staticmethod
    def backward(ctx, g):
        zeros = tuple(torch.zeros(sh, dtype=torch.float32, device=dev) for sh, _, dev in ctx.shapes)
        return (g,) + zeros


def touch_zero_grad(t, params):
    return _ZeroGradTouch.apply(t, *params)


class _FanOut(Function):
    @staticmethod
    def forward(ctx, x, n, token, step=None, events=None):
        ctx.n, ctx.token, ctx.step, ctx.events = n, token, step, events
        ctx.set_materialize_grads(False)
        return tuple(x.view_as(x) for _ in range(n))

    @staticmethod
    def backward(ctx, *grads):
        if ctx.events:
            cur = torch.cuda.current_stream()
            for ev in ctx.events.values():
                cur.wait_event(ev)
            ctx.events.clear()
# ... 2 lines not shown
            if grads[i] is None:
                raise RuntimeError(f"scanpaths_amd: fan-out alias {i} recorded a split-only gradient but no gradient arrived for it")
        idx = [i for i, g in enumerate(grads) if g is not None]
        if not idx:
            return None, None, None, None, None
        for i in idx:
            if i not in tok and getattr(grads[i], "_sp_skipped", False):
                raise RuntimeError("scanpaths_amd: a gradient whose fp32 form was left unwritten reached a fan-in without its record")
        gs = [grads[i].contiguous() for i in idx]
        ops = [tok.get(i) for i in idx]
        tok.clear()
        if any(op is not None for op in ops):
            out = torch.empty_like(gs[0])
            n = out.numel()
            assert n % 16 == 0 and len(gs) <= 32, (n, len(gs))
            f = (C.c_void_p * len(gs))(*[None if op is not None else g.data_ptr() for g, op in zip(gs, ops)])
            pl = (C.c_void_p * len(gs))(*[op.buf.data_ptr() if op is not None else None for op in ops])
            sc = (C.c_void_p * len(gs))(*[op.scale.data_ptr() if op is not None else None for op in ops])
            hint = _amax_hint(out.device)
            rcs = [op.rows[0] for op in ops if op is not None and op.rows is not None]
            rc = rcs[0] if (rcs and all(r is rcs[0] for r in rcs) and (n // rcs[0].B) % 16 == 0 and n % rcs[0].B == 0) else None
            steps = (C.c_int * len(gs))(*[(op.rows[1] if (op is not None and op.rows is not None) else -1) for op in ops]) if rc else None
            check(hip.lib().sp_sum_n_mixed(f, pl, sc, len(gs), n, ptr(out), _hint_ptr(hint), ptr(rc.last) if rc else None, steps,
                                           rc.B if rc else 0, hip.stream()), "sp_sum_n_mixed")
            if hint is not None:
                out._sp_amax = hint
            return out, None, None, None, None
        if len(gs) == 1:
            return gs[0], None, None, None, None
        out = torch.empty_like(gs[0])
        n = out.numel()
        if n % 4 or len(gs) > 32:
            acc = gs[0]
            for g in gs[1:]:
                acc = _add_raw(acc, g)
            return acc, None, None, None, None
        arr = (C.c_void_p * len(gs))(*[g.data_ptr() for g in gs])
        hint = _amax_hint(out.device)
        rc0 = rows_ctx(ctx.step, gs[0].shape[0]) if gs[0].dim() > 1 else None
        marks = [getattr(grads[i], "_sp_rows", None) for i in idx]
        if rc0 is None and any(m is not None for m in marks):
            cand = next(m[0] for m in marks if m is not None)
            if gs[0].dim() > 1 and cand.B == gs[0].shape[0] and ROW_SPARSITY:
                rc0 = cand
        steps = None
        if rc0 is not None and n % rc0.B == 0 and (n // rc0.B) % 4 == 0:
            if ctx.step is not None:
                steps = [int(ctx.step)] * len(gs)
            else:
                steps = [int(m[1]) if (m is not None and m[0] is rc0) else -1 for m in marks]
        sparse = steps is not None and any(st >= 0 for st in steps)
        if sparse:
            FUSION_COUNTS["fan_in_rows"] += 1
        check(hip.lib().sp_sum_n(arr, len(gs), n, ptr(out), _hint_ptr(hint), ptr(rc0.last) if sparse else None,
                                 (C.c_int * len(gs))(*steps) if sparse else None, rc0.B if sparse else 0, hip.stream()), "sp_sum_n")
        if hint is not None:
            out._sp_amax = hint
        return out, None, None, None, None


def fanout(x: torch.Tensor, n: int, step=None):
    split_ok = x.numel() % 16 == 0 and n <= 32
    token = {} if split_ok else None
    events = {} if (ASYNC_DGRAD and step is not None and x.is_cuda) else None
    outs = _FanOut.apply(x, n, token, step, events)
    if events is not None:
        for i, o in enumerate(outs):
            o._sp_fan_ev = (events, i)
    for attr in ("_sp_cache", "_sp_amax"):
        v = getattr(x, attr, None)
        if v is not None:
            for o in outs:
                setattr(o, attr, v)
    if split_ok:
        for i, o in enumerate(outs):
            o._sp_fan = (token, i)
            o._sp_split_grad_ok = True
    return outs




class GradMerge:
    __slots__ = ("first", "merged")

    def __init__(self):
        self.first, self.merged = None, False


class _Tap(Function):
    @staticmethod
    def forward(ctx, x, holder):
        ctx.holder = holder
        return x.view_as(x), x.view_as(x)

    @staticmethod
    def backward(ctx, g_main, g_side):
        h = ctx.holder
        merged, h.first, h.merged = h.merged, None, False
        if g_main is None or g_side is None:
            return (g_main if g_side is None else g_side), None
        if merged:
            return g_main, None
        return _add_raw(g_main.contiguous(), g_side.contiguous()), None


def tap(x: torch.Tensor, holder: GradMerge):
    outs = _Tap.apply(x, holder)
    for attr in ("_sp_cache", "_sp_amax"):
        v = getattr(x, attr, None)
        if v is not None:
            for o in outs:
                setattr(o, attr, v)
    return outs


class _ScaleConst(Function):
    @staticmethod
    def forward(ctx, x, c):
        x = x.contiguous()
        ctx.c = float(c)
        cs = torch.full((1,), float(c), dtype=torch.float32, device=x.device)
        out = torch.empty_like(x)
        check(hip.lib().sp_scale_by(ptr(x), ptr(cs), x.numel(), ptr(out), hip.stream()), "sp_scale_by")
        return out

    @staticmethod
    def backward(ctx, g):
        return _ScaleConst.apply(g, ctx.c), None


def scale_const(x: torch.Tensor, c: float) -> torch.Tensor:
    return _ScaleConst.apply(x, c)


def add(a: torch.Tensor, b: torch.Tensor) -> torch.Tensor:
    return _Add.apply(a, b)


def _phys(w: torch.Tensor) -> torch.Tensor:
    p = w.permute(0, 2, 3, 1)
    return p if p.is_contiguous() else p.contiguous()


class _Conv2d(Function):
    @staticmethod
    def forward(ctx, x, w, bias, stride, pad, dil, relu, wcache=None, bn_stats=False, grad_store=None, grad_accum=None, step=None):
        ctx.grad_store, ctx.grad_accum, ctx.step = grad_store, grad_accum, step
        ctx.w_param = _grad_slot(w) if w.dim() == 4 else None
        defer = wcache.get("defer") if isinstance(wcache, dict) else None
        ctx.defer_final = defer.claim() if (defer is not None and ctx.needs_input_grad[1]) else False
        ctx.dy_token = None
        x = x.contiguous()
        wp = _phys(w.detach())
        assert wp.shape[3] == x.shape[3], (wp.shape, x.shape)
        need_dx, need_dw = ctx.needs_input_grad[:2]
        g = ConvGeom.of(x.shape, *wp.shape[:3], stride, pad, dil)
        y = torch.empty((g.N, g.Ho, g.Wo, g.Co), dtype=torch.float32, device=x.device)
        shared = getattr(x, "_sp_cache", None) is not None
        if getattr(x, "_sp_uninit", False) and not conv_runs_from_split(x.shape, w, stride, pad, dil, need_dw):
            raise RuntimeError("scanpaths_amd: a BatchNorm left this input's fp32 form unwritten (skip_z) but this conv does not run "
                               "from the split operand alone; run with SP_BN_SKIP_DX=0")
        xs, stats = _conv_fwd(g, x, wp, bias, y, relu=relu, wcache=wcache, channel=True, free_a=shared, a_elems=x.numel(), bn_stats=bn_stats)
        if xs is not None:
            y._sp_from_split = xs.scheme == "f16x2"
            if stats is not None:
                FUSION_COUNTS["conv_bn_stats"] += 1
                y._sp_bnstats = stats
            keep = need_dw and g.wgrad_split(free_splits=True) == xs.scheme
            if (y._sp_from_split and g.wgrad_scheme == "f16x2" and bias is None and not relu and (not need_dw or keep)
                    and (not need_dx or g.dgrad_split(free_a=True, a_elems=y.numel()))):
                ctx.dy_token = y._sp_dy_token = {"skipped": False}
            if not keep:
                xs = None
        ctx.xs_scheme = (xs.scheme, xs.kind) if xs is not None else None
        xs_buf, xs_scale = (xs.buf, xs.scale) if xs is not None else (None, None)
        ctx.geom, ctx.cfg = g, (relu, bias is not None)
        ctx.wcache = wcache
        ctx.save_for_backward(x, wp, y if relu else None, xs_buf, xs_scale)
        return y

    @staticmethod
    def backward(ctx, dy):
        relu, has_bias = ctx.cfg
        x, wp, y, xs_buf, xs_scale = ctx.saved_tensors
        xs = SplitOperand(xs_buf, xs_scale, *ctx.xs_scheme) if xs_buf is not None else None
        if ctx.dy_token is not None and ctx.dy_token["skipped"] and getattr(dy, "_sp_cache", None) is None:
            raise RuntimeError("scanpaths_amd: a BatchNorm left this gradient's fp32 form unwritten (skip_dx) but its split form "
                               "did not arrive with it; run with SP_BN_SKIP_DX=0")
        dy = dy.contiguous()
        if relu:
            dyr = torch.empty_like(dy)
            check(hip.lib().sp_relu_bwd(ptr(dy), ptr(y), dy.numel(), ptr(dyr), hip.stream()), "sp_relu_bwd")
            dy = dyr
        dx, dw = _conv_backward(ctx.geom, x, wp, dy, xs, ctx.wcache, ctx.needs_input_grad[0], ctx.needs_input_grad[1],
                                accum=ctx.grad_accum, defer_final=ctx.defer_final, step=ctx.step, w_param=ctx.w_param)
        if ctx.grad_store is not None and dx is not None:
            ctx.grad_store.first = dx
        db = _colsum_any(dy, wp.shape[0]) if (has_bias and ctx.needs_input_grad[2]) else None
        return dx, dw, db, None, None, None, None, None, None, None, None, None




class DeferredWgrad:
    __slots__ = ("items", "claimed")

    def __init__(self):
        self.items, self.claimed = [], False

    def claim(self) -> bool:
        first, self.claimed = not self.claimed, True
        return first


def _flush_deferred(defer, wp, g: ConvGeom):
    items, defer.items, defer.claimed = defer.items, [], False
    if all(st is not None for _, _, st in items):
        items = sorted(items, key=lambda it: it[2])
    dwp = torch.empty_like(wp)
    L = hip.lib()
    xs0, dys0, _ = items[0]
    same = all(x.kind == xs0.kind and y.kind == dys0.kind for x, y, _ in items)
    steps = [st for _, _, st in items]
    toks = [getattr(st, "rows", None) for st in steps]
    rc = rows_ctx(steps[0], g.N) if (toks and toks[0] is not None and all(tk is toks[0] for tk in toks)) else None
    d = g.wgrad_desc(x_scale_vec=int(xs0.kind == "cols"), y_scale_vec=int(dys0.kind == "cols"))
    nseg = len(items)
    wsb = L.sp_conv_wgrad_f16x2_multi_workspace(C.byref(d), nseg) if (same and not THROUGHPUT_MODE and 1 < nseg <= 16) else 0
    if wsb > 0:
        ws = hip.workspace(wsb, wp.device, slot=3)
        arr = lambda ts: (C.c_void_p * nseg)(*[t.data_ptr() for t in ts])
        Xa, Sxa = arr([x.buf for x, _, _ in items]), arr([x.scale for x, _, _ in items])
        Ya, Sya = arr([y.buf for _, y, _ in items]), arr([y.scale for _, y, _ in items])
        seg_steps = (C.c_int * nseg)(*steps) if rc is not None else None
        if rc is not None:
            FUSION_COUNTS["row_sparse_bwd"] += 1

        def launch():
            check(L.sp_conv_wgrad_f16x2_multi(C.byref(d), nseg, Xa, Sxa, Ya, Sya, ptr(dwp), ptr(ws), ptr(rc.last) if rc is not None else None,
                                              seg_steps, hip.stream()), "sp_conv_wgrad_f16x2_multi")
        FUSION_COUNTS["wgrad_multi"] += 1
        _timed(lambda: (("h2_wgrad_multi" + ("_rows" if rc is not None else ""), g.M * nseg, g.Co, g.K, f"{g.KH}x{g.KW}", nseg),
                        2.0 * g.M * nseg * g.Co * g.K), launch)
    else:
        for k, (x, y, _) in enumerate(items):
            _wgrad_b3(g.wgrad_desc(beta=int(k > 0)), x, y, dwp)
    return dwp.permute(0, 3, 1, 2)


def _conv_backward(g: ConvGeom, x, wp, dy, xs, wcache, need_dx, need_dw, accum=None, defer_final=False, step=None, w_param=None):
    dx = dw = None
    dys = None
    dy_cached = getattr(dy, "_sp_cache", None)
    defer = wcache.get("defer") if (DEFER_WGRAD and isinstance(wcache, dict)) else None
    rc = rows_ctx(step, g.N)
    deferred = False
    if need_dw and defer is not None:
        wsch = g.wgrad_scheme
        have = dy_cached is not None and wsch in dy_cached
        if wsch == "f16x2" and xs is not None and xs.scheme == wsch and g.wgrad_split(free_splits=have):
            dys = dy_cached[wsch] if have else split_op(dy, wsch, channel=True)
            defer.items.append((xs, dys, step))
            deferred = True
    if need_dx:
        beta = 0
        if accum is not None and accum.first is not None and accum.first.shape == x.shape and accum.first.is_contiguous():
            dx, beta, accum.merged = accum.first, 1, True
            FUSION_COUNTS["grad_merge"] += 1
        else:
            dx = torch.empty_like(x)
        dys = _conv_dgrad(g, dy, wp, dx, dys=dys, wcache=wcache, channel=True, free_a=dy_cached is not None or dys is not None,
                          a_elems=dy.numel(), beta=beta, rows=(rc, step) if rc is not None else None) or dys
    slot = None
    if need_dw and not deferred:
        if defer is None:
            slot, dwp = _take_grad_view(w_param, (0, 2, 3, 1))
        if slot is None:
            dwp = torch.empty_like(wp)
        _conv_wgrad(g, x, dy, dwp, xs=xs, dys=dys, channel=True)
        if slot is not None:
            slot.done()
        else:
            dw = dwp.permute(0, 3, 1, 2)
    if need_dw and defer is not None and defer_final and defer.items:
        dsum = _flush_deferred(defer, wp, g)
        dw = dsum if dw is None else dw + dsum
    return dx, dw


def _geom_of_logical(x_shape, w, stride=1, pad=0, dil=1) -> ConvGeom:
    return ConvGeom.of(x_shape, w.shape[0], w.shape[2], w.shape[3], stride, pad, dil)


def conv_takes_split(x_shape, w, stride=1, pad=0, dil=1) -> bool:
    g = _geom_of_logical(x_shape, w, stride, pad, dil)
    return _scheme_for(g.Ci) == "f16x2" and g.fwd_split(free_a=True, a_elems=g.N * g.H * g.W * g.Ci)


def conv_runs_from_split(x_shape, w, stride=1, pad=0, dil=1, need_dw=True) -> bool:
    if not conv_takes_split(x_shape, w, stride, pad, dil):
        return False
    return (not need_dw) or _geom_of_logical(x_shape, w, stride, pad, dil).wgrad_split(free_splits=True) == "f16x2"


def conv2d(x, w, bias=None, stride=1, pad=0, dil=1, relu=False, wcache=None, bn_stats=False, grad_store=None, grad_accum=None, step=None):
    return _Conv2d.apply(x, w, bias, stride, pad, dil, relu, wcache, bn_stats, grad_store, grad_accum, step)


class _PadLast(Function):
    @staticmethod
    def forward(ctx, x, cout):
        x = x.contiguous()
        cin = x.shape[-1]
        rows = x.numel() // cin
        y = torch.empty(x.shape[:-1] + (cout,), dtype=torch.float32, device=x.device)
        check(hip.lib().sp_pad_lastdim(ptr(x), rows, cin, cout, ptr(y), hip.stream()), "sp_pad_lastdim")
        ctx.cin = cin
        return y

    @staticmethod
    def backward(ctx, dy):
        dy = dy.contiguous()
        cout = dy.shape[-1]
        rows = dy.numel() // cout
        dx = torch.empty(dy.shape[:-1] + (ctx.cin,), dtype=torch.float32, device=dy.device)
        check(hip.lib().sp_pad_lastdim(ptr(dy), rows, cout, ctx.cin, ptr(dx), hip.stream()), "sp_pad_lastdim")
        return dx, None


def pad_last(x, cout):
    return _PadLast.apply(x, cout)


def nchw_to_nhwc(x: torch.Tensor, cpad: int) -> torch.Tensor:
    x = x.contiguous()
    N, Cc, H, W_ = x.shape
    y = torch.empty((N, H, W_, cpad), dtype=torch.float32, device=x.device)
    check(hip.lib().sp_nchw_to_nhwc_pad(ptr(x), N, Cc, H, W_, cpad, ptr(y), hip.stream()), "sp_nchw_to_nhwc_pad")
    return y


def _rows(t):
    assert t.stride(-1) == 1
    if t.dim() == 2:
        return 1, t.shape[0], t.shape[1], t.stride(0), 0
    assert t.dim() == 3
    return t.shape[0], t.shape[1], t.shape[2], t.stride(1), t.stride(0)


class DeferredGemmWgrad:
    __slots__ = ("items", "claimed")

    def __init__(self):
        self.items, self.claimed = [], False

# ... 97 lines not shown
        invstd = torch.empty(Cc, dtype=torch.float32, device=dev)
        if training:
            ws = hip.workspace(L.sp_bn_workspace(M, Cc), dev, slot=1)
            check(L.sp_bn_stats(ptr(x), M, Cc, eps, momentum, ptr(mean), ptr(invstd), ptr(rmean), ptr(rvar), ptr(ws),
                                hip.stream()), "sp_bn_stats")
        else:
            check(L.sp_bn_eval_stats(ptr(rmean), ptr(rvar), Cc, eps, ptr(mean), ptr(invstd), hip.stream()),
                  "sp_bn_eval_stats")
        y = torch.empty_like(x)
        res = residual.contiguous() if residual is not None else None
        hint = _amax_hint(dev)
        check(L.sp_bn_apply(ptr(x), ptr(mean), ptr(invstd), ptr(gamma), ptr(beta), ptr(res), int(relu), M, Cc, ptr(y),
                            _hint_ptr(hint), hip.stream()), "sp_bn_apply")
        if hint is not None:
            y._sp_amax = hint
        ctx.cfg = (training, relu, residual is not None)
        ctx.save_for_backward(x, y if relu else None, mean, invstd, gamma.detach())
        return y

    @staticmethod
    def backward(ctx, dy):
        training, relu, has_res = ctx.cfg
        x, y, mean, invstd, gamma = ctx.saved_tensors
        dy = dy.contiguous()
        Cc = x.shape[-1]
        M = x.numel() // Cc
        L = hip.lib()
        dx = torch.empty_like(x)
        dres = torch.empty_like(x) if has_res else None
        dgamma = torch.empty(Cc, dtype=torch.float32, device=x.device)
        dbeta = torch.empty(Cc, dtype=torch.float32, device=x.device)
        ws = hip.workspace(L.sp_bn_workspace(M, Cc), x.device, slot=1)
        hint = _amax_hint(x.device)
        check(L.sp_bn_backward(ptr(dy), ptr(x), ptr(y), ptr(mean), ptr(invstd), ptr(gamma), int(relu), int(training), M, Cc,
                               ptr(dx), ptr(dres), ptr(dgamma), ptr(dbeta), ptr(ws), _hint_ptr(hint), hip.stream()),
              "sp_bn_backward")
        if hint is not None:
            dx._sp_amax = hint
        return dx, dgamma, dbeta, None, None, dres, None, None, None, None




class _BnActSplit(Function):
    @staticmethod
    def forward(ctx, x, gamma, beta, rmean, rvar, residual, momentum, eps, relu, emit_fwd, emit_bwd, pre, res_store=None,
                dy_token=None, skip_z=False):
        ctx.res_store = res_store
        ctx.params = (_grad_slot(gamma), _grad_slot(beta))
        ctx.dy_token = dy_token
        x = x.contiguous()
        Cc = x.shape[-1]
        M = x.numel() // Cc
        n = x.numel()
        L = hip.lib()
        dev = x.device
        mean = torch.empty(Cc, dtype=torch.float32, device=dev)
        invstd = torch.empty(Cc, dtype=torch.float32, device=dev)
        ext = torch.empty(2 * Cc, dtype=torch.float32, device=dev)
        ws = hip.workspace(L.sp_bn_split_workspace(M, Cc), dev, slot=1)
        emit_fwd = bool(emit_fwd) and Cc % 16 == 0
        planes = torch.empty(2 * n + 32, dtype=torch.float16, device=dev) if emit_fwd else None
        mask = torch.empty(L.sp_bn_mask_words(M, Cc), dtype=torch.int64, device=dev) if relu else None
        y = torch.empty_like(x)
        res = residual.contiguous() if residual is not None else None
        zhint, bhint = _amax_hint(dev), _amax_hint(dev)
        skip_z = bool(skip_z) and planes is not None
        check(L.sp_bn_fwd_split(ptr(x), M, Cc, eps, momentum, ptr(gamma), ptr(beta), ptr(res),
                                _hint_ptr(residual._sp_amax) if residual is not None else None, int(relu), ptr(mean), ptr(invstd),
                                ptr(rmean), ptr(rvar), ptr(ext), None if skip_z else ptr(y), ptr(planes), ptr(zhint),
                                _hint_ptr(bhint), ptr(mask),
                                ptr(ws), ptr(pre[0]) if pre else None, ptr(pre[1]) if pre else None, pre[2] if pre else 0,
                                hip.stream()), "sp_bn_fwd_split")
        y._sp_amax = zhint
        FUSION_COUNTS["bn_fwd_split"] += 1
        if planes is not None:
            FUSION_COUNTS["bn_fwd_split_operand"] += 1
            y._sp_cache = {"f16x2": SplitOperand(planes, zhint, "f16x2")}
        if skip_z:
            FUSION_COUNTS["bn_skip_z"] += 1
            y._sp_uninit = True
        ctx.cfg = (relu, residual is not None, bool(emit_bwd) and Cc % 16 == 0)
        ctx.save_for_backward(x, mask, mean, invstd, gamma.detach(), ext)
        return y

    @staticmethod
    def backward(ctx, dy):
        relu, has_res, emit = ctx.cfg
        x, mask, mean, invstd, gamma, ext = ctx.saved_tensors
        dy = dy.contiguous()
        Cc = x.shape[-1]
        M = x.numel() // Cc
        L = hip.lib()
        dev = x.device
        dx = torch.empty_like(x)
        dres = torch.empty_like(x) if has_res else None
        gslot, dgamma = _take_grad_view(ctx.params[0]) if ctx.needs_input_grad[1] else (None, None)
        bslot, dbeta = _take_grad_view(ctx.params[1]) if ctx.needs_input_grad[2] else (None, None)
        if dgamma is None:
            dgamma = torch.empty(Cc, dtype=torch.float32, device=dev)
        if dbeta is None:
            dbeta = torch.empty(Cc, dtype=torch.float32, device=dev)
        planes = torch.empty(2 * x.numel() + 32, dtype=torch.float16, device=dev) if emit else None
        ws = hip.workspace(L.sp_bn_split_workspace(M, Cc), dev, slot=1)
        dhint, bhint = _amax_hint(dev), _amax_hint(dev)
        skip = emit and ctx.dy_token is not None
        FUSION_COUNTS["bn_bwd_split"] += 1
        if emit:
            FUSION_COUNTS["bn_bwd_split_operand"] += 1
        if skip:
            FUSION_COUNTS["bn_skip_dx"] += 1
            ctx.dy_token["skipped"] = True
        check(L.sp_bn_bwd_split(ptr(dy), ptr(x), ptr(mask), ptr(mean), ptr(invstd), ptr(gamma), ptr(ext), M, Cc,
                                None if skip else ptr(dx),
                                ptr(dres), ptr(planes), ptr(dhint), _hint_ptr(bhint), ptr(dgamma), ptr(dbeta), ptr(ws),
                                hip.stream()), "sp_bn_bwd_split")
        dx._sp_amax = dhint
        if planes is not None:
            dx._sp_cache = {"f16x2": SplitOperand(planes, dhint, "f16x2")}
        if ctx.res_store is not None and dres is not None:
            ctx.res_store.first = dres
        if gslot is not None:
            gslot.done()
            dgamma = None
        if bslot is not None:
            bslot.done()
            dbeta = None
        return dx, dgamma, dbeta, None, None, dres, None, None, None, None, None, None, None, None, None




def bn_act(x, gamma, beta, rmean, rvar, residual=None, training=True, momentum=0.1, eps=1e-5, relu=True, emit_split=False,
           res_store=None, skip_dx=False, skip_z=False):
    if (training and BN_SPLIT and x.shape[-1] % 4 == 0 and _amax_hint_active()
            and (residual is None or getattr(residual, "_sp_amax", None) is not None)):
        emit_bwd = getattr(x, "_sp_from_split", False)
        token = getattr(x, "_sp_dy_token", None) if (skip_dx and BN_SKIP_DX and emit_bwd) else None
        return _BnActSplit.apply(x, gamma, beta, rmean, rvar, residual, momentum, eps, relu, emit_split, emit_bwd,
                                 getattr(x, "_sp_bnstats", None), res_store, token, skip_z and emit_split and BN_SKIP_DX and BN_SKIP_Z)
    return _BnAct.apply(x, gamma, beta, rmean, rvar, residual, training, momentum, eps, relu)


class _MaxPool(Function):
    @staticmethod
    def forward(ctx, x):
        x = x.contiguous()
        N, H, W_, Cc = x.shape
        Ho = -(-(H - 3) // 2) + 1
        Wo = -(-(W_ - 3) // 2) + 1
        if (Ho - 1) * 2 >= H:
            Ho -= 1
        if (Wo - 1) * 2 >= W_:
            Wo -= 1
        y = torch.empty((N, Ho, Wo, Cc), dtype=torch.float32, device=x.device)
        amx = torch.empty((N, Ho, Wo, Cc), dtype=torch.uint8, device=x.device) if ctx.needs_input_grad[0] else None
        check(hip.lib().sp_maxpool3s2_fwd(ptr(x), N, H, W_, Cc, ptr(y), ptr(amx), Ho, Wo, hip.stream()), "sp_maxpool3s2_fwd")
        ctx.shape = (N, H, W_, Cc, Ho, Wo)
        ctx.save_for_backward(amx)
        return y

    @staticmethod
    def backward(ctx, dy):
        (amx,) = ctx.saved_tensors
        dy = dy.contiguous()
        N, H, W_, Cc, Ho, Wo = ctx.shape
        dx = torch.empty((N, H, W_, Cc), dtype=torch.float32, device=dy.device)
        check(hip.lib().sp_maxpool3s2_bwd(ptr(dy), ptr(amx), N, H, W_, Cc, ptr(dx), Ho, Wo, hip.stream()), "sp_maxpool3s2_bwd")
        return dx


def maxpool3s2(x):
    return _MaxPool.apply(x)


class _GateConv(Function):
    @staticmethod
    def forward(ctx, h, w_h, spcol, wc, hw):
        spcol = spcol.contiguous()
        wc = wc.contiguous()
        B, P, KP = spcol.shape
        N3 = wc.shape[1]
        wp = _phys(w_h.detach())
        C4 = wp.shape[0]
        if h is not None:
            h = h.contiguous()
            g = ConvGeom.of((B,) + h.shape[1:], C4, 3, 3, pad=1)
            hg = torch.empty((B, g.H, g.W, C4), dtype=torch.float32, device=spcol.device)
            _conv_fwd(g, h, wp, None, hg)
        else:
            hg = torch.zeros((B, hw[0], hw[1], C4), dtype=torch.float32, device=spcol.device)
        _igemm(_gemm_desc(P, N3, KP, ldx=KP, ldw=KP, ldc=C4, beta=1, nbatch=B, sX=P * KP, sW=N3 * KP, sC=P * C4), spcol, wc, None, hg)
        ctx.has_h = h is not None
        ctx.save_for_backward(h, wp, spcol, wc)
        return hg

    @staticmethod
    def backward(ctx, dhg):
        h, wp, spcol, wc = ctx.saved_tensors
        dhg = dhg.contiguous()
        B, P, KP = spcol.shape
        N3 = wc.shape[1]
        C4 = wp.shape[0]
# ... 860 lines not shown
```

scanpaths_amd/hip.py:

```python
from __future__ import annotations

import ctypes as C
import os
from typing import Optional

import torch

from . import config as _config

_HERE = os.path.dirname(os.path.abspath(__file__))
TIMING_LIB = False
LIB_PATH = ""


def _apply_config():
    global TIMING_LIB, LIB_PATH
    TIMING_LIB = _config.settings["library"] == "timing"
    LIB_PATH = os.path.join(_HERE, "libscanpaths_amd_timing.so" if TIMING_LIB else "libscanpaths_amd.so")


_apply_config()


class ConvDesc(C.Structure):
    _fields_ = [("N_img", C.c_int), ("Hi", C.c_int), ("Wi", C.c_int), ("Kc", C.c_int), ("ldx", C.c_int),
                ("Ho", C.c_int), ("Wo", C.c_int), ("Nout", C.c_int), ("ldc", C.c_int),
                ("KH", C.c_int), ("KW", C.c_int), ("stride", C.c_int), ("pad", C.c_int), ("dil", C.c_int),
                ("mode", C.c_int), ("ldw", C.c_int),
                ("alpha", C.c_float), ("beta", C.c_int), ("relu", C.c_int),
                ("nbatch", C.c_int),
                ("strideX", C.c_int64), ("strideW", C.c_int64), ("strideC", C.c_int64),
                ("ksplit", C.c_int), ("workspace", C.c_void_p), ("w_scale_rows", C.c_int),
                ("row_last", C.c_void_p), ("row_step", C.c_int)]


class WgradDesc(C.Structure):
    _fields_ = [("N_img", C.c_int), ("Hi", C.c_int), ("Wi", C.c_int), ("Ci", C.c_int), ("ldx", C.c_int),
                ("Ho", C.c_int), ("Wo", C.c_int), ("Co", C.c_int), ("ldy", C.c_int),
                ("KH", C.c_int), ("KW", C.c_int), ("stride", C.c_int), ("pad", C.c_int), ("dil", C.c_int),
                ("ldo", C.c_int), ("beta", C.c_int), ("alpha", C.c_float), ("nbatch", C.c_int),
                ("strideX", C.c_int64), ("strideY", C.c_int64), ("strideO", C.c_int64),
                ("x_scale_vec", C.c_int), ("y_scale_vec", C.c_int), ("row_last", C.c_void_p), ("row_step", C.c_int)]


_P, _I, _L, _F = C.c_void_p, C.c_int, C.c_int64, C.c_float
ABI_VERSION = 4

SIGNATURES = {
    "sp_abi_version": (_I, []),
    "sp_set_tuning": (_I, [C.c_char_p, _I]),
    "sp_timing_build": (_I, []),
    "sp_conv_igemm": (_I, [C.POINTER(ConvDesc), _P, _P, _P, _P, _P]),
    "sp_split3_bf16": (_I, [_P, _L, _P, _P]),
    "sp_split3_bf16_wT": (_I, [_P, _I, _I, _I, _P, _P]),
    "sp_split2_f16": (_I, [_P, _L, _P, _P, _I, _P]),
    "sp_split2_f16_wT": (_I, [_P, _I, _I, _I, _P, _P, _P]),
    "sp_split2_f16_rows": (_I, [_P, _L, _L, _I, _P, _P, _P, _P]),
    "sp_split2_f16_wT_rows": (_I, [_P, _I, _I, _I, _I, _P, _P, _P, _P]),
    "sp_split2_f16_cols_workspace": (_L, [_L, _I]),
    "sp_split2_f16_cols": (_I, [_P, _L, _I, _P, _P, _P, _P]),
    "sp_conv_wgrad_f16x2_multi_workspace": (_L, [_P, _I]),
    "sp_conv_wgrad_f16x2_multi": (_I, [_P, _I, _P, _P, _P, _P, _P, _P, _P, _P, _P]),
    "sp_conv_igemm_f16x2": (_I, [_P, _P, _P, _P, _P, _P, _P, _P]),
    "sp_conv_wgrad_f16x2_workspace": (_L, [_P]),
    "sp_conv_wgrad_f16x2": (_I, [_P, _P, _P, _P, _P, _P, _P, _P]),
    "sp_conv_igemm_f16x1": (_I, [_P, _P, _P, _P, _P, _P, _P, _P]),
    "sp_conv_wgrad_f16x1": (_I, [_P, _P, _P, _P, _P, _P, _P, _P]),
    "sp_gateconv_lstm_f16x2": (_I, [_P, _P, _P, _P, _P, _P, _P, _P, _P, _I, _I, _P, _P, _P, _P, _P, _P, _F, _P]),
    "sp_rank1_grads_applies": (_I, [_I, _I, _I, _I, _I]),
    "sp_rank1_grads_workspace": (_L, [_I, _I, _I, _I]),
    "sp_rank1_grads_f16x2": (_I, [_P, _P, _I, _P, _P, _P, _I, _I, _I, _I, _P, _P, _P, _P, _I, _P]),
    "sp_conv_igemm_bf16x3": (_I, [C.POINTER(ConvDesc), _P, _P, _P, _P, _P]),
    "sp_conv_wgrad_bf16x3_workspace": (_L, [C.POINTER(WgradDesc)]),
    "sp_conv_wgrad_bf16x3": (_I, [C.POINTER(WgradDesc), _P, _P, _P, _P, _P]),
    "sp_conv_wgrad_workspace": (_L, [C.POINTER(WgradDesc)]),
    "sp_conv_wgrad": (_I, [C.POINTER(WgradDesc), _P, _P, _P, _P, _P]),
    "sp_colsum_workspace": (_L, [_L, _I]),
    "sp_colsum": (_I, [_P, _L, _I, _I, _P, _I, _P, _P]),
    "sp_rowsum": (_I, [_P, _L, _I, _F, _P, _P]),
    "sp_rowsum_bwd": (_I, [_P, _L, _I, _F, _P, _P]),
    "sp_bn_workspace": (_L, [_L, _I]),
    "sp_bn_stats": (_I, [_P, _L, _I, _F, _F, _P, _P, _P, _P, _P, _P]),
    "sp_bn_eval_stats": (_I, [_P, _P, _I, _F, _P, _P, _P]),
    "sp_bn_apply": (_I, [_P, _P, _P, _P, _P, _P, _I, _L, _I, _P, _P, _P]),
    "sp_bn_backward": (_I, [_P, _P, _P, _P, _P, _P, _I, _I, _L, _I, _P, _P, _P, _P, _P, _P, _P]),
    "sp_bn_split_workspace": (_L, [_L, _I]),
    "sp_bn_mask_words": (_L, [_L, _I]),
    "sp_bn_fwd_split": (_I, [_P, _L, _I, _F, _F, _P, _P, _P, _P, _I, _P, _P, _P, _P, _P, _P, _P, _P, _P, _P, _P, _P, _P, _I, _P]),
    "sp_conv_stats_tiles": (_L, [C.POINTER(ConvDesc)]),
    "sp_conv_igemm_f16x2_stats": (_I, [C.POINTER(ConvDesc), _P, _P, _P, _P, _P, _P, _P, _P]),
    "sp_bn_bwd_split": (_I, [_P, _P, _P, _P, _P, _P, _P, _L, _I, _P, _P, _P, _P, _P, _P, _P, _P, _P]),
    "sp_sum_n": (_I, [_P, _I, _L, _P, _P, _P, _P, _I, _P]),
    "sp_sum_n_mixed": (_I, [_P, _P, _P, _I, _L, _P, _P, _P, _P, _I, _P]),
    "sp_relu_bwd": (_I, [_P, _P, _L, _P, _P]),
    "sp_maxpool3s2_fwd": (_I, [_P, _I, _I, _I, _I, _P, _P, _I, _I, _P]),
    "sp_maxpool3s2_bwd": (_I, [_P, _P, _I, _I, _I, _I, _P, _I, _I, _P]),
    "sp_nchw_to_nhwc_pad": (_I, [_P, _I, _I, _I, _I, _I, _P, _P]),
    "sp_pad_lastdim": (_I, [_P, _L, _I, _I, _P, _P]),
    "sp_add": (_I, [_P, _P, _P, _L, _P]),
    "sp_lstm_pointwise_fwd": (_I, [_P, _P, _P, _L, _I, _P, _P, _P, _P]),
    "sp_lstm_rank1_fwd": (_I, [_P, _P, _P, _P, _P, _I, _I, _I, _I, _P, _P, _P, _P, _P]),
    "sp_rank1_dwc_workspace": (_L, [_I, _I, _I, _I]),
    "sp_rank1_dwc": (_I, [_P, _P, _I, _I, _I, _I, _I, _P, _P, _P]),
    "sp_sempool_workspace": (_L, [_I, _I, _I, _I]),
    "sp_sempool_fwd": (_I, [_P, _P, _I, _I, _I, _I, _F, _P, _P, _I, _P]),
    "sp_sempool_bwd": (_I, [_P, _P, _P, _P, _I, _I, _I, _I, _F, _P, _P, _P, _I, _I, _P]),
    "sp_lstm_pointwise_bwd": (_I, [_P, _P, _P, _P, _P, _L, _I, _P, _P, _P, _P, _P, _P, _F, _F, _P, _P, _P, _I, _I, _P]),
    "sp_im2col3x3_1ch": (_I, [_P, _I, _I, _I, _I, _I, _P, _P]),
    "sp_col2im3x3_1ch": (_I, [_P, _I, _I, _I, _I, _I, _P, _P]),
    "sp_listatt_fwd": (_I, [_P, _P, _I, _I, _I, _P, _P, _P]),
    "sp_listatt_bwd": (_I, [_P, _P, _P, _P, _I, _I, _I, _P, _P, _P]),
    "sp_mulrelu_fwd": (_I, [_P, _P, _L, _L, _P, _P]),
    "sp_mulrelu_bwd": (_I, [_P, _P, _P, _P, _L, _L, _P, _P, _P]),
    "sp_select_rows": (_I, [_P, _P, _P, _L, _L, _P, _P]),
    "sp_select_rows_bwd": (_I, [_P, _P, _L, _L, _P, _P, _P]),
    "sp_head_finish_fwd": (_I, [_P, _I, _I, _I, _I, _I, _I, _P, _I, _P, _P, _I, _P, _P, _P, _P, _P, _P, _I, _I, _P]),
    "sp_head_finish_bwd": (_I, [_P, _L, _P, _P, _P, _P, _P, _P, _P, _I, _I, _I, _I, _I, _I, _P, _I, _P, _P, _P, _P, _P, _I,
                                _I, _P, _P]),
    "sp_head_num_classes": (_I, [_I, _I]),
    "sp_head_compose11_fwd": (_I, [_P, _P, _I, _I, _I, _I, _I, _P, _P, _P]),
    "sp_head_compose11_bwd": (_I, [_P, _P, _I, _I, _I, _I, _I, _P, _P, _P]),
    "sp_sal_gather_fwd": (_I, [_P, _I, _I, _I, _I, _I, _P, _P, _P]),
    "sp_sal_gather_bwd": (_I, [_P, _I, _I, _I, _I, _I, _I, _P, _P, _P, _I, _P]),
    "sp_drt_direct_fwd": (_I, [_P, _P, _P, _P, _I, _I, _I, _I, _I, _P, _P]),
    "sp_drt_direct_bwd_data": (_I, [_P, _P, _P, _I, _I, _I, _I, _I, _I, _P, _P, _P, _I, _I, _P]),
    "sp_drt_direct_bwd_weight_workspace": (_L, [_I, _I, _I, _I, _I]),
    "sp_drt_direct_bwd_weight": (_I, [_P, _P, _P, _I, _I, _I, _I, _I, _I, _P, _P, _P, _P, _P, _I, _I, _P]),
    "sp_scanmatch_max_len": (_I, []),
    "sp_scanmatch_submatrix": (_I, [_I, _I, C.c_double, _P, _P, _P]),
    "sp_scanmatch_sequences": (_I, [_P, _I, _P, _P, _I, _I, _I, _I, _I, C.c_double, C.c_double, C.c_double, _P, _I, _P, _P, _P]),
    "sp_scanmatch_score": (_I, [_P, _P, _I, _P, _P, _I, _P, _I, _P, _I, _P, C.c_double, _P, _P]),
    "sp_scanmatch_score_long_workspace": (_L, [_I, _I]),
    "sp_scanmatch_score_long": (_I, [_P, _P, _I, _P, _P, _I, _P, _I, _P, _I, _P, C.c_double, _P, _P, _P]),
    "sp_scanmatch_align": (_I, [_P, _I, _P, _I, _P, _I, _P, C.c_double, _P, _P, _P, _P, _P, _P]),
    "sp_scan_max_fixations": (_I, []),
    "sp_scan_sed_stde": (_I, [_P, _I, _P, _P, _P, _I, _I, _I, _I, C.c_double, _P, _P, _P]),
    "sp_scan_tde": (_I, [_P, _I, _P, _P, _P, _I, _I, _I, C.c_double, _P, _P, _P]),
    "sp_scan_multimatch": (_I, [_P, _I, _P, _P, _P, _I, C.c_double, C.c_double, _P, _P]),
    "sp_scan_simplify": (_I, [_P, _I, _P, _P, _I, C.c_double, C.c_double, C.c_double, _P, _P, _P]),
    "sp_scan_multimatch_gated": (_I, [_P, _I, _P, _P, _P, _P, _I, C.c_double, C.c_double, _P, _P]),
    "sp_scan_distances": (_I, [_P, _I, _P, _P, _P, _I, C.c_double, _P, _P, _P, _P, _P]),
    "sp_scan_recurrence": (_I, [_P, _I, _P, _P, _P, _I, C.c_double, C.c_double, _I, _P, _P]),
    "sp_meanshift_max_points": (_I, []),
    "sp_meanshift": (_I, [_P, _I, _P, _P, _I, C.c_double, _I, _P, _P, _P, _P, _P]),
    "sp_scan_cluster_strings": (_I, [_P, _I, _P, _P, _P, _I, _P, _P, _P, _P, _P]),
    "sp_scan_sequence": (_I, [_P, _P, _P, _P, _I, C.c_double, _P, _P, _P]),
    "sp_sample_actions": (_I, [_P, _P, _P, _I, _I, _I, _I, C.c_uint64, _P, _P, _P, _P]),
    "sp_generate_scanpath": (_I, [_P, _P, _I, _I, _I, _I, _I, _I, _P, _P, _P, _P, _P, _P]),
    "sp_beam_search": (_I, [_P, _I, _I, _I, _I, _I, _P, _P, _P]),
    "sp_collate_targets": (_I, [_P, _P, _P, _P, _P, _P, _P, _P, _I, _I, _I, _I, _I, _P, _P, _P, _P, _P]),
    "sp_blur_targets": (_I, [_P, _I, _I, _I, C.c_double, _P]),
    "sp_scanpath_loss_workspace": (_L, [_I, _I]),
    "sp_scanpath_loss": (_I, [_P, _P, _P, _P, _P, _P, _P, _I, _I, _I, _F, _P, _P, _P, _P, _P, _P, _P]),
    "sp_log_action": (_I, [_P, _P, _I, _I, _P, _P, _P, _P]),
    "sp_log_duration": (_I, [_P, _P, _P, _P, _I, _I, _P, _P, _P, _P, _P]),
    "sp_rowscale": (_I, [_P, _P, _I, _I, _P, _P]),
    "sp_rows_last": (_I, [_P, _P, _I, _I, _I, _I, _P, _P]),
    "sp_gemm_skinny_applies": (_I, [_I, _I, _I, _I, _I, _I, _I]),
    "sp_gemm_skinny_workspace": (_L, [_I, _I, _I, _I]),
    "sp_gemm_skinny": (_I, [_P, _P, _P, _P, _I, _I, _I, _I, _I, _I, _I, _F, _I, _P, _P]),
    "sp_scale_by": (_I, [_P, _P, _L, _P, _P]),
    "sp_sumsq_workspace": (_L, [_L]),
    "sp_sum": (_I, [_P, _L, _P, _P, _P]),
    "sp_sumsq": (_I, [_P, _L, _P, _P, _P]),
    "sp_smooth_l1_loss": (_I, [_P, _P, _P, _L, _P, _P, _P]),
    "sp_rayleigh_loss": (_I, [_P, _P, _P, _L, _P, _P, _P]),
    "sp_abs_diff_mean": (_I, [_P, _P, _L, _P, _P, _P, _P]),
    "sp_nss_loss": (_I, [_P, _P, _I, _I, _P, _P, _P, _P, _P]),
    "sp_cc_loss": (_I, [_P, _P, _I, _I, _P, _P, _P, _P, _P]),
    "sp_kld_loss": (_I, [_P, _P, _I, _I, _P, _P, _P, _P, _P]),
    "sp_cc_terms": (_I, [_P, _P, _P, _P, _I, _I, _I, _P, _P, _P, _P, _P]),
    "sp_kld_box_alignment": (_I, [_P, _P, _P, _I, _P, _P, _I, _I, _I, _P, _P, _P, _P, _P]),
    "sp_kld_question_alignment": (_I, [_P, _P, _P, _P, _I, _I, _I, _I, _P, _P, _P, _P, _P, _P]),
    "sp_rowscale_idx": (_I, [_P, _P, _P, _I, _I, _P, _P]),
# ... 136 lines not shown
```

scanpaths_amd/models/scanpath_model.py:

```python
from __future__ import annotations

from typing import Dict, List, Optional

import torch
import torch.nn as nn

from .. import functional as F
from ..spec import ARCHS, COCO_OBJECTS, drt_hw, encoder_channels

HC = 64
NTAP = 49


class _Conv(nn.Module):
    def __init__(self, cin, cout, kh, kw=None, bias=True):
        super().__init__()
        kw = kh if kw is None else kw
        self.weight = nn.Parameter(torch.empty(cout, cin, kh, kw).contiguous(memory_format=torch.channels_last))
        if bias:
            self.bias = nn.Parameter(torch.zeros(cout))
        else:
            self.register_parameter("bias", None)


# ... 122 lines not shown
            self.object_sal_layer = nn.ModuleDict({k: _Conv(512, 512, 5) for k in self.object_name})
        self.object_head = _Head(Hm, Wm)
        self.last_decode_rows = None
        self.init_weights()

    def _replicate_for_data_parallel(self):
        raise RuntimeError(
            "scanpaths_amd: this model cannot be replicated by nn.DataParallel (its parameters are views of the optimiser's flat "
            "buffers and its HIP kernels use per-process workspaces).  Pass a single id in --gpu_ids (the reference's default is "
            "[0, 1], AiR/opts.py:26), or run one process per GPU: `python -m torch.distributed.run --nproc-per-node N "
            "--master-addr 127.0.0.1 train.py` with scanpaths_amd.ddp (shard_batch, global_mask_normaliser, broadcast_module_state_) "
            "and scanpaths_amd.optim.FlatAdam -- see INTEGRATION.md, 'multi-GPU'.")

    def init_weights(self):
        for name, m in self.named_modules():
            if isinstance(m, _Conv):
                co, ci, kh, kw = m.weight.shape
                if name.startswith("resnet."):
                    nn.init.normal_(m.weight, 0.0, (2.0 / (kh * kw * co)) ** 0.5)
                else:
                    nn.init.xavier_normal_(m.weight)
                    if m.bias is not None:
                        nn.init.zeros_(m.bias)
            elif isinstance(m, _Linear):
                nn.init.normal_(m.weight, 0.0, 0.01)
                nn.init.zeros_(m.bias)

    def _bn(self, bn: _BN, x, residual=None, relu=True, emit_split=False, res_store=None, skip_z=False):
        y = F.bn_act(x, bn.weight, bn.bias, bn.running_mean, bn.running_var, residual, training=self.training, relu=relu,
                     emit_split=emit_split, res_store=res_store, skip_dx=True, skip_z=skip_z)
        if self.training:
            self._bn_seen.append(bn.num_batches_tracked)
        return y

    def encode(self, images):
        r = self.resnet
        self._bn_seen = []
        x = F.nchw_to_nhwc(images, 4)
        w0 = F.pad_last(r[0].weight.permute(0, 2, 3, 1), 4).permute(0, 3, 1, 2)
        x = F.conv2d(x, w0, None, stride=2, pad=3)
        x = self._bn(r[1], x)
        st = self.training
        x = F.maxpool3s2(x)
        kind = ARCHS[self.arch][0]
        blocks = []
        for li in range(4):
            first_stride = 2 if li == 2 else 1
            dil = {2: 2, 3: 4}.get(li, 1)
            for bi, blk in enumerate(r[4 + li]):
                blocks.append((blk, first_stride if bi == 0 else 1, dil))
        for k, (blk, s, dil) in enumerate(blocks):
            gm = F.GradMerge() if (F.GRAD_MERGE and torch.is_grad_enabled() and x.requires_grad) else None
            x, x_side = F.tap(x, gm) if gm is not None else (x, x)
            if kind == "bottleneck":
                o = F.conv2d(x, blk.conv1.weight, None, stride=s, bn_stats=st, grad_accum=gm)
                o = self._bn(blk.bn1, o, emit_split=F.conv_takes_split(o.shape, blk.conv2.weight, pad=dil, dil=dil),
                             skip_z=F.conv_runs_from_split(o.shape, blk.conv2.weight, pad=dil, dil=dil,
                                                           need_dw=blk.conv2.weight.requires_grad))
                o = F.conv2d(o, blk.conv2.weight, None, pad=dil, dil=dil, bn_stats=st)
                o = self._bn(blk.bn2, o, emit_split=F.conv_takes_split(o.shape, blk.conv3.weight),
                             skip_z=F.conv_runs_from_split(o.shape, blk.conv3.weight, need_dw=blk.conv3.weight.requires_grad))
                o = F.conv2d(o, blk.conv3.weight, None, bn_stats=st)
                last = blk.bn3
            else:
                o = F.conv2d(x, blk.conv1.weight, None, stride=s, pad=1, bn_stats=st, grad_accum=gm)
                o = self._bn(blk.bn1, o, emit_split=F.conv_takes_split(o.shape, blk.conv2.weight, pad=dil, dil=dil))
                o = F.conv2d(o, blk.conv2.weight, None, pad=dil, dil=dil, bn_stats=st)
                last = blk.bn2
            idn = x_side
            if blk.downsample is not None:
                idn = self._bn(blk.downsample[1], F.conv2d(x_side, blk.downsample[0].weight, None, stride=s, bn_stats=st,
                                                           grad_store=gm), relu=False)
            if k + 1 < len(blocks):
                nb, ns, _ = blocks[k + 1]
                emit = F.conv_takes_split(o.shape, nb.conv1.weight, stride=ns, pad=0 if kind == "bottleneck" else 1) or \
                    (nb.downsample is not None and F.conv_takes_split(o.shape, nb.downsample[0].weight, stride=ns))
            else:
                emit = True
            x = self._bn(last, o, residual=idn, relu=True, emit_split=emit,
                         res_store=gm if blk.downsample is None else None)
        if self._bn_seen:
            torch._foreach_add_(self._bn_seen, 1)
        self._bn_seen = []
        return x

    @staticmethod
    def _cat_phys(ws: List[torch.Tensor]) -> torch.Tensor:
        return torch.cat([w.permute(0, 2, 3, 1) for w in ws], 0).permute(0, 3, 1, 2)

    def _sum_bias(self, names):
        b = getattr(self.lstm, names[0]).bias
        for n in names[1:]:
            b = F.add(b, getattr(self.lstm, n).bias)
        return b

    def _compose_heads(self, convs: List[_Conv]):
        oh = self.object_head
        dev = oh.sal_layer_2.weight.device
        z = lambda *s: torch.zeros(*s, dtype=torch.float32, device=dev)
        wcomp = torch.cat([oh.sal_layer_2.weight.view(1, 512), oh.sal_layer_3.weight.view(1, 512),
                           oh.drt_layer_1.weight.permute(0, 2, 3, 1).reshape(NTAP, 512), z(HC - 2 - NTAP, 512)], 0)
        own = torch.cat([oh.sal_layer_2.bias, oh.sal_layer_3.bias, z(NTAP), oh.drt_layer_1.bias, z(HC - 3 - NTAP)])
        Gs, cbs = [], []
        for cv in convs:
            w5 = cv.weight.permute(0, 2, 3, 1).reshape(512, 25 * 512)
            Gs.append(F.gemm(wcomp, w5, None, "kn"))
            b4 = torch.cat([cv.bias.view(1, 512), z(3, 512)], 0)
            cbs.append(F.add(F.gemm(wcomp, b4, None, "nk")[:, 0].contiguous(), own))
        G = torch.cat(Gs, 0).view(len(convs) * HC, 5, 5, 512).permute(0, 3, 1, 2)
        return G, torch.stack(cbs, 0)

    def _attention_vectors(self):
        sa, pa = self.semantic_att, self.spatial_att
        dev = sa.semantic_lists.weight.device
        u_sem = F.gemm(sa.semantic_attention.weight, sa.semantic_lists.weight, None, "kn").view(512)
        Hm, Wm = self.map_height, self.map_width
        acol = F.im2col3x3(pa.spatial_attention.weight.view(1, 1, Hm, Wm), 12).view(Hm * Wm, 12)
        wl = torch.cat([pa.spatial_lists.weight.reshape(9).flip(0), torch.zeros(3, device=dev)]).view(1, 12)
        wl4 = torch.cat([wl, torch.zeros(3, 12, device=dev)], 0)
        u_spa = F.gemm(acol, wl4, None, "nk")[:, 0].contiguous()
        u_sem = F.touch_zero_grad(u_sem, [sa.semantic_lists.bias, sa.semantic_cur.weight, sa.semantic_cur.bias,
                                          sa.semantic_attention.bias])
        u_spa = F.touch_zero_grad(u_spa, [pa.spatial_lists.bias, pa.spatial_cur.weight, pa.spatial_cur.bias,
                                          pa.spatial_attention.bias])
        return u_sem, u_spa

    def _heads_prepare(self, B, Hm, Wm, dev, tasks=None):
        S = len(self.streams)
        if self.task == "AiR":
            head_convs = [self.performance_sal_layer["True"], self.performance_sal_layer["False"]]
        elif self.task == "OSIE":
            head_convs = [self.performance_sal_layer]
        else:
            head_convs = None
        nh = S
        if head_convs is not None:
            G, cb = self._compose_heads(head_convs)
            cbt = None
            nsrc, per_sample = len(head_convs), False
            hmap = torch.arange(nh, dtype=torch.int32, device=dev).repeat(B, 1).contiguous()
        else:
            tl = [int(t) for t in tasks.tolist()]
            uniq = sorted(set(tl))
            G, cbt = self._compose_heads([self.object_sal_layer[self.int2object[t]] for t in uniq])
            slot = torch.tensor([uniq.index(t) for t in tl], device=dev)
            cb = cbt.index_select(0, slot).view(B, 1, HC)
            nsrc, per_sample = len(uniq), True
            hmap = slot.to(torch.int32).view(B, 1).contiguous()
        Gp = G.permute(0, 2, 3, 1).reshape(nsrc, HC, 25, 512)
        R = (nsrc * 50 + 63) // 64 * 64
        Wsal = torch.cat([Gp[:, :2].reshape(nsrc * 50, 512), torch.zeros(R - nsrc * 50, 512, device=dev)], 0).view(R, 512, 1, 1)
        W11, cbsum = F.compose11(G, cbt if per_sample else cb, nsrc, HC, (Hm, Wm))
        return dict(nh=nh, nsrc=nsrc, per_sample=per_sample, hmap=hmap, Wsal=Wsal, W11=W11, cbsum=cbsum, cb=cb,
                    w2=self.object_head.drt_layer_2.weight, b2=self.object_head.drt_layer_2.bias)

    def _heads_step(self, hp, h_sal, h_drt, Wsal, W11, cbsum, cb, w2, b2, step=None):
        Z2 = F.sal_gather(F.conv2d(h_sal, Wsal, None, pad=0, step=step), hp["hmap"], hp["nh"], hp["nsrc"], step=step)
        Dpre = F.drt_direct(h_drt, W11, cbsum, hp["hmap"], hp["nh"], step=step)
        return F.head_finish(Z2, cb, w2, b2, hp["nh"], HC, not self.training, per_sample=hp["per_sample"], dpre=Dpre)

    def decode(self, enc, attention_maps, tasks=None):
        T = self.convLSTM_length
        S = len(self.streams)
        grad_on_outer = torch.is_grad_enabled()
        vf = F.conv2d(enc, self.sal_conv.weight, self.sal_conv.bias, pad=1, relu=True)
        B, Hm, Wm, Cc = vf.shape
# ... 128 lines not shown
```

Before: 137.7 images/s.

## Fold BN backward reductions and lazy residual add into conv dgrad epilogue

Extends the f16x2 implicit-GEMM data-gradient epilogue so that, while storing dx, it also computes the per-tile BatchNorm backward partial sums (sum dy, sum dy*xhat, max |dy|) for the preceding BN. The BN backward kernel then consumes these precomputed partials instead of re-reading dy and x. It also defers the residual-branch gradient: instead of materialising dres and summing it later, the masked residual dy is added inside the conv1 dgrad epilogue. The aim is to cut full-tensor memory passes in the ResNet backward. In exchange the epilogue gains extra register pressure, global loads and a block barrier, and the Python side gains considerable bookkeeping and validity checks.

```diff
diff --git a/include/scanpaths_amd.h b/include/scanpaths_amd.h
--- a/include/scanpaths_amd.h
+++ b/include/scanpaths_amd.h
@@ -80,6 +80,18 @@
 int64_t sp_conv_stats_tiles(const sp_conv_desc* d);
 int sp_conv_igemm_f16x2_stats(const sp_conv_desc* d, const void* Xsplit, const float* x_scale, const void* Wsplit,
                               const float* w_scale, float* out, double* st_partial, float* st_mm, void* stream);
+typedef struct sp_bn_fold {
+    const float* x;
+    const unsigned long long* mask;
+    const float* mean;
+    const float* invstd;
+    double* partial;
+    float* dmax;
+    const float* res_dy;
+    const unsigned long long* res_mask;
+} sp_bn_fold;
+int sp_conv_igemm_f16x2_bnbwd(const sp_conv_desc* d, const void* Xsplit, const float* x_scale, const void* Wsplit,
+                              const float* w_scale, float* out, const sp_bn_fold* fold, void* stream);
 int sp_conv_igemm_f16x1(const sp_conv_desc* d, const void* Xsplit, const float* x_scale, const void* Wsplit, const float* w_scale,
                         const float* bias, float* out, void* stream);
 int sp_conv_wgrad_f16x1(const sp_wgrad_desc* d, const void* Xsplit, const float* x_scale, const void* dYsplit,
@@ -125,7 +137,9 @@
                     const float* pre_mm , int pre_G, void* stream);
 int sp_bn_bwd_split(const float* dy, const float* x, const unsigned long long* mask, const float* mean, const float* invstd,
                     const float* gamma, const float* ext, int64_t M, int C, float* dx, float* dres, void* planes, float* dx_scale,
-                    unsigned* bound, float* dgamma, float* dbeta, void* workspace, void* stream);
+                    unsigned* bound, float* dgamma, float* dbeta, void* workspace,
+                    const double* pre_partial ,
+                    const float* pre_dmax , int pre_G, void* stream);
 
 int sp_maxpool3s2_fwd(const float* x, int N, int H, int W, int C, float* y, unsigned char* argmax , int Ho, int Wo,
                       void* stream);
diff --git a/scanpaths_amd/config.py b/scanpaths_amd/config.py
--- a/scanpaths_amd/config.py
+++ b/scanpaths_amd/config.py
@@ -5,7 +5,7 @@
 
 DEFAULTS = {
     "split_scheme": "f16x2", "use_split": True, "library": "product", "always_reset_amax": False,
-    "fused_amax": True, "grad_merge": True, "bn_split": True, "bn_skip_dx": True, "bn_skip_z": True, "lstm_bwd_split": True,
+    "fused_amax": True, "grad_merge": True, "bn_split": True, "bn_skip_dx": True, "bn_skip_z": True, "bn_bwd_fold": True, "lstm_bwd_split": True,
     "rank1_dsp_split": True, "rank1_dwc_split": True, "lstm_skip_dpre": True, "fuse_gate_lstm": True, "lstm_h_planes": True,
     "defer_wgrad": True, "channel_scales": True, "hw2_single": True, "row_sparsity": True, "direct_grad": True, "skinny_gemm": True, "async_dgrad": True,
     "drt_batched": True, "rank1_fused": True,
@@ -15,7 +15,7 @@
     "SP_SPLIT_SCHEME": ("split_scheme", str), "SP_NO_SPLIT": ("use_split", lambda v: not v), "SP_LIBRARY": ("library", str),
     "SP_ALWAYS_RESET_AMAX": ("always_reset_amax", bool), "SP_NO_AMAX_HINT": ("fused_amax", lambda v: not v),
     "SP_GRAD_MERGE": ("grad_merge", _off), "SP_BN_SPLIT": ("bn_split", _off), "SP_BN_SKIP_DX": ("bn_skip_dx", _off),
-    "SP_BN_SKIP_Z": ("bn_skip_z", _off), "SP_LSTM_BWD_SPLIT": ("lstm_bwd_split", _off), "SP_RANK1_DSP_SPLIT": ("rank1_dsp_split", _off),
+    "SP_BN_SKIP_Z": ("bn_skip_z", _off), "SP_BN_BWD_FOLD": ("bn_bwd_fold", _off), "SP_LSTM_BWD_SPLIT": ("lstm_bwd_split", _off), "SP_RANK1_DSP_SPLIT": ("rank1_dsp_split", _off),
     "SP_RANK1_DWC_SPLIT": ("rank1_dwc_split", _off), "SP_LSTM_SKIP_DPRE": ("lstm_skip_dpre", _off), "SP_FUSE_LSTM": ("fuse_gate_lstm", _off),
     "SP_LSTM_H_PLANES": ("lstm_h_planes", _off), "SP_DEFER_WGRAD": ("defer_wgrad", _off), "SP_CHANNEL_SCALES": ("channel_scales", _off),
     "SP_HW2_SINGLE": ("hw2_single", _off), "SP_ROW_SPARSITY": ("row_sparsity", _off), "SP_DIRECT_GRAD": ("direct_grad", _off), "SP_SKINNY_GEMM": ("skinny_gemm", _off),
diff --git a/scanpaths_amd/csrc/bn_pool.hip b/scanpaths_amd/csrc/bn_pool.hip
--- a/scanpaths_amd/csrc/bn_pool.hip
+++ b/scanpaths_amd/csrc/bn_pool.hip
@@ -958,23 +958,28 @@
 extern "C" int sp_bn_bwd_split(const float* dy, const float* x, const unsigned long long* mask, const float* mean,
                                const float* invstd, const float* gamma, const float* ext, int64_t M, int C, float* dx,
                                float* dres, void* planes, float* dx_scale, unsigned* bound, float* dgamma, float* dbeta,
-                               void* workspace, void* stream) {
+                               void* workspace, const double* pre_partial, const float* pre_dmax, int pre_G, void* stream) {
     if (!dy || !x || !mean || !invstd || !gamma || !ext || !dx_scale || !bound || !dgamma || !dbeta || !workspace) return SP_ENULL;
     if (!dx && !planes) return SP_ENULL;
     if (C % 4 || (planes && C % 16) || M <= 0 || ((uintptr_t)planes & 15)) return SP_EINVAL;
+    if (pre_partial && (!pre_dmax || pre_G < 1)) return SP_EINVAL;
     hipStream_t s = (hipStream_t)stream;
     const bool wide = C >= 256 && C % 256 == 0;
-    const int G = wide ? pick_G_wide(M, C) : pick_G(M, C);
-    double* partial = (double*)workspace;
-    float* dmax = (float*)(partial + (int64_t)G * 2 * C);
-    float* coef = dmax + (int64_t)G * 2 * C;
+    int G = wide ? pick_G_wide(M, C) : pick_G(M, C);
+    const double* partial = (double*)workspace;
+    const float* dmax = (float*)((double*)workspace + (int64_t)G * 2 * C);
+    float* coef = (float*)dmax + (int64_t)G * 2 * C;
     SP_RESET_AMAX(bound, s);
-    if (wide)
+    if (pre_partial) {
+        partial = pre_partial;
+        dmax = pre_dmax;
+        G = pre_G;
+    } else if (wide)
         hipLaunchKernelGGL(bn_bwd_mm_partial<64>, dim3((unsigned)(C / 256), G), dim3(256), 0, s, dy, x, mask, mean, invstd, M, C, G,
-                           partial, dmax);
+                           (double*)partial, (float*)dmax);
     else
         hipLaunchKernelGGL(bn_bwd_mm_partial<16>, dim3((unsigned)sp_cdiv(C, CB), G), dim3(256), 0, s, dy, x, mask, mean, invstd, M, C,
-                           G, partial, dmax);
+                           G, (double*)partial, (float*)dmax);
     SP_LAUNCH_CHECK();
     if (G > 256)
         hipLaunchKernelGGL((bn_bwd_mm_final<8, 32>), dim3((unsigned)sp_cdiv(C, 8)), dim3(256), 0, s, partial, dmax, M, C, G, gamma,
diff --git a/scanpaths_amd/csrc/conv_f16x2.hip b/scanpaths_amd/csrc/conv_f16x2.hip
--- a/scanpaths_amd/csrc/conv_f16x2.hip
+++ b/scanpaths_amd/csrc/conv_f16x2.hip
@@ -59,7 +59,20 @@
     const int* row_last;
     int row_step;
     int row_nimg;
+    const float* bb_x;
+    const unsigned long long* bb_mask;
+    const float* bb_mean;
+    const float* bb_invstd;
+    double* bb_partial;
+    float* bb_dmax;
+    const float* res_dy;
+    const unsigned long long* res_mask;
 };
+
+template <int K>
+__device__ __forceinline__ unsigned quad_bcast(unsigned v) {
+    return (unsigned)__builtin_amdgcn_mov_dpp((int)v, K * 0x55, 0xf, 0xf, true);
+}
 
 __device__ __forceinline__ float h2_sigmoid(float x) { return sp_sigmoid(x); }
 __device__ __forceinline__ int halo_swz(int slot) { return ((slot >> 1) & 3) << 1; }
@@ -788,7 +801,116 @@
             if (full_m && n0 + HBN <= p.Nout && !p.relu) {
                 float* dst0 = p.C + (m0 + wm * 64 + rsub) * p.ldc + n;
                 const float* src0 = stg + rsub * 68 + 4 * cq4;
-                if (!p.beta) {
+                bool bb = false, res = false;
+                if constexpr (MODE == 1 && !LSTM) {
+                    bb = p.bb_partial != nullptr;
+                    res = p.res_dy != nullptr;
+                }
+                if (bb || res) {
+                    if constexpr (MODE == 1 && !LSTM) {
+                        const int64_t e0 = (m0 + wm * 64 + rsub) * (int64_t)p.ldc + n;
+                        float4 mu = make_float4(0.f, 0.f, 0.f, 0.f), is = mu;
+                        if (bb) {
+                            mu = *reinterpret_cast<const float4*>(p.bb_mean + n);
+                            is = *reinterpret_cast<const float4*>(p.bb_invstd + n);
+                        }
+                        const float m4[4] = {mu.x, mu.y, mu.z, mu.w}, i4[4] = {is.x, is.y, is.z, is.w};
+                        const bool bmask = bb && p.bb_mask != nullptr, rmask = res && p.res_mask != nullptr;
+                        double s1[4] = {0.0, 0.0, 0.0, 0.0}, s2[4] = {0.0, 0.0, 0.0, 0.0};
+                        float mx[4] = {0.f, 0.f, 0.f, 0.f};
+                        auto mask_piece = [&](const unsigned long long* mask, int64_t e) -> unsigned {
+                            const int64_t i = e >> 2;
+                            return reinterpret_cast<const unsigned short*>(mask + (i >> 6) * 4)[(lane & 3) * 4 + (int)((i & 63) >> 4)];
+                        };
+#pragma unroll
+                        for (int h = 0; h < 2; ++h) {
+                            float4 xv[8], ov[8], rv[8];
+                            unsigned bm[8], rm[8];
+#pragma unroll
+                            for (int q = 0; q < 8; ++q) {
+                                const int64_t e = e0 + (int64_t)((h * 8 + q) * 4) * p.ldc;
+                                xv[q] = ov[q] = rv[q] = make_float4(0.f, 0.f, 0.f, 0.f);
+                                bm[q] = rm[q] = 0xffffu;
+                                if (bb) xv[q] = *reinterpret_cast<const float4*>(p.bb_x + e);
+                                if (p.beta) ov[q] = *reinterpret_cast<const float4*>(p.C + e);
+                                if (res) rv[q] = *reinterpret_cast<const float4*>(p.res_dy + e);
+                                if (bmask) bm[q] = mask_piece(p.bb_mask, e);
+                                if (rmask) rm[q] = mask_piece(p.res_mask, e);
+                            }
+#pragma unroll
+                            for (int q = 0; q < 8; ++q) {
+                                const int ps = h * 8 + q;
+                                const int bit = (int)((e0 >> 2) & 15);
+                                const float4 sv = *reinterpret_cast<const float4*>(src0 + ps * 4 * 68);
+                                float v[4] = {sv.x, sv.y, sv.z, sv.w};
+                                const float o[4] = {ov[q].x, ov[q].y, ov[q].z, ov[q].w}, r[4] = {rv[q].x, rv[q].y, rv[q].z, rv[q].w};
+                                const float a[4] = {xv[q].x, xv[q].y, xv[q].z, xv[q].w};
+                                unsigned bw[4] = {0xffffu, 0xffffu, 0xffffu, 0xffffu}, rw[4] = {0xffffu, 0xffffu, 0xffffu, 0xffffu};
+                                if (bmask) {
+                                    bw[0] = quad_bcast<0>(bm[q]); bw[1] = quad_bcast<1>(bm[q]);
+                                    bw[2] = quad_bcast<2>(bm[q]); bw[3] = quad_bcast<3>(bm[q]);
+                                }
+                                if (rmask) {
+                                    rw[0] = quad_bcast<0>(rm[q]); rw[1] = quad_bcast<1>(rm[q]);
+                                    rw[2] = quad_bcast<2>(rm[q]); rw[3] = quad_bcast<3>(rm[q]);
+                                }
+#pragma unroll
+                                for (int k = 0; k < 4; ++k) {
+                                    if (p.beta) v[k] += o[k];
+                                    if (res) v[k] += ((rw[k] >> bit) & 1u) ? r[k] : 0.f;
+                                }
+                                *reinterpret_cast<float4*>(p.C + e0 + (int64_t)(ps * 4) * p.ldc) = make_float4(v[0], v[1], v[2], v[3]);
+                                if (bb) {
+#pragma unroll
+                                    for (int k = 0; k < 4; ++k) {
+                                        const float d = ((bw[k] >> bit) & 1u) ? v[k] : 0.f;
+                                        s1[k] += (double)d;
+                                        s2[k] += (double)(d * (a[k] - m4[k]) * i4[k]);
+                                        mx[k] = fmaxf(mx[k], fabsf(d));
+                                    }
+                                }
+                            }
+                        }
+                        if (bb) {
+#pragma unroll
+                            for (int k = 0; k < 4; ++k)
+#pragma unroll
+                                for (int off = 16; off <= 32; off <<= 1) {
+                                    s1[k] += __shfl_xor(s1[k], off);
+                                    s2[k] += __shfl_xor(s2[k], off);
+                                    mx[k] = fmaxf(mx[k], __shfl_xor(mx[k], off));
+                                }
+                            double* sh_s = reinterpret_cast<double*>(smem + 8 * 64 * 68 * sizeof(float));
+                            float* sh_m = reinterpret_cast<float*>(sh_s + 3 * HBN * 2);
+                            const int col = wn * 64 + 4 * cq4;
+                            if (wm > 0 && rsub == 0) {
+#pragma unroll
+                                for (int k = 0; k < 4; ++k) {
+                                    sh_s[((wm - 1) * HBN + col + k) * 2 + 0] = s1[k];
+                                    sh_s[((wm - 1) * HBN + col + k) * 2 + 1] = s2[k];
+                                    sh_m[(wm - 1) * HBN + col + k] = mx[k];
+                                }
+                            }
+                            asm volatile("s_waitcnt lgkmcnt(0)" ::: "memory");
+                            __builtin_amdgcn_s_barrier();
+                            if (wm == 0 && rsub == 0) {
+                                const int64_t g = m0 / HBM;
+#pragma unroll
+                                for (int k = 0; k < 4; ++k) {
+#pragma unroll
+                                    for (int w = 0; w < 3; ++w) {
+                                        s1[k] += sh_s[(w * HBN + col + k) * 2 + 0];
+                                        s2[k] += sh_s[(w * HBN + col + k) * 2 + 1];
+                                        mx[k] = fmaxf(mx[k], sh_m[w * HBN + col + k]);
+                                    }
+                                    p.bb_partial[(g * 2 + 0) * p.Nout + n + k] = s1[k];
+                                    p.bb_partial[(g * 2 + 1) * p.Nout + n + k] = s2[k];
+                                }
+                                *reinterpret_cast<float4*>(p.bb_dmax + g * p.Nout + n) = make_float4(mx[0], mx[1], mx[2], mx[3]);
+                            }
+                        }
+                    }
+                } else if (!p.beta) {
 #pragma unroll
                     for (int ps = 0; ps < 16; ++ps)
                         *reinterpret_cast<float4*>(dst0 + (int64_t)(ps * 4) * p.ldc) = *reinterpret_cast<const float4*>(src0 + ps * 4 * 68);
@@ -1871,7 +1993,7 @@
 
 static int conv_igemm_f16(const sp_conv_desc* d, const void* Xs, const float* x_scale, const void* Ws, const float* w_scale,
                           const float* bias, float* out, void* stream, int nprod, double* st_partial = nullptr,
-                          float* st_mm = nullptr) {
+                          float* st_mm = nullptr, const sp_bn_fold* bf = nullptr) {
     if (!d || !Xs || !Ws || !x_scale || !w_scale || !out) return SP_ENULL;
     if (d->mode != 0 && d->mode != 1) return SP_EINVAL;
     if (d->Kc % 32 || d->ldx < d->Kc || d->ldx % 16) return SP_EINVAL;
@@ -1912,6 +2034,22 @@
         a.st_partial = st_partial; a.st_mm = st_mm;
         return cbm_ok ? launch_h2<0, 3, true>(a, st) : launch_h2<0, 3, false>(a, st);
     }
+    if (bf) {
+        const bool sums = bf->partial != nullptr;
+        if (!sums && !bf->res_dy) return SP_ENULL;
+        if (sums && (!bf->x || !bf->mean || !bf->invstd || !bf->dmax)) return SP_ENULL;
+        if (f || d->nbatch != 1 || nprod != 3 || a.M % HBM || d->Nout % HBN || d->ldc != d->Nout || d->relu || bias || a.row_last)
+            return SP_EINVAL;
+        if (bf->res_dy && d->beta) return SP_EINVAL;
+        if (((uintptr_t)out | (uintptr_t)bf->x | (uintptr_t)bf->mask | (uintptr_t)bf->mean | (uintptr_t)bf->invstd |
+             (uintptr_t)bf->partial | (uintptr_t)bf->dmax | (uintptr_t)bf->res_dy | (uintptr_t)bf->res_mask) & 15)
+            return SP_EINVAL;
+        if (sums) {
+            a.bb_x = bf->x; a.bb_mask = bf->mask; a.bb_mean = bf->mean; a.bb_invstd = bf->invstd;
+            a.bb_partial = bf->partial; a.bb_dmax = bf->dmax;
+        }
+        a.res_dy = bf->res_dy; a.res_mask = bf->res_dy ? bf->res_mask : nullptr;
+    }
 #ifdef SP_TIMING_VARIANTS
     if (sp_tuning_get(SP_TUNE_H2_DBG, 0) >= 256) a.l_probe = sp_tuning_get(SP_TUNE_H2_DBG, 0) & ~255;
     switch (sp_tuning_get(SP_TUNE_H2_DBG, 0)) {
@@ -1943,6 +2081,12 @@
                                          const float* w_scale, float* out, double* st_partial, float* st_mm, void* stream) {
     if (!st_partial || !st_mm) return SP_ENULL;
     return conv_igemm_f16(d, Xs, x_scale, Ws, w_scale, nullptr, out, stream, 3, st_partial, st_mm);
+}
+
+extern "C" int sp_conv_igemm_f16x2_bnbwd(const sp_conv_desc* d, const void* Xs, const float* x_scale, const void* Ws,
+                                         const float* w_scale, float* out, const sp_bn_fold* fold, void* stream) {
+    if (!fold) return SP_ENULL;
+    return conv_igemm_f16(d, Xs, x_scale, Ws, w_scale, nullptr, out, stream, 3, nullptr, nullptr, fold);
 }
 
 extern "C" int sp_conv_igemm_f16x1(const sp_conv_desc* d, const void* Xs, const float* x_scale, const void* Ws,
diff --git a/scanpaths_amd/functional.py b/scanpaths_amd/functional.py
--- a/scanpaths_amd/functional.py
+++ b/scanpaths_amd/functional.py
@@ -9,7 +9,7 @@
 
 from . import config as _config
 from . import hip
-from .hip import ConvDesc, WgradDesc, check, ptr
+from .hip import BnFold, ConvDesc, WgradDesc, check, ptr
 
 
 _KSPLIT_MIN_NKT, _KSPLIT_KT = 8, 4
@@ -74,6 +74,7 @@
     g["THROUGHPUT_MODE"] = c["split_scheme"] == "f16x1"
     g["SPLIT_SCHEME"] = "f16x2" if c["split_scheme"] == "f16x1" else c["split_scheme"]
     for name, key in (("GRAD_MERGE", "grad_merge"), ("BN_SPLIT", "bn_split"), ("BN_SKIP_DX", "bn_skip_dx"), ("BN_SKIP_Z", "bn_skip_z"),
+                      ("BN_BWD_FOLD", "bn_bwd_fold"),
                       ("LSTM_BWD_SPLIT", "lstm_bwd_split"), ("RANK1_DSP_SPLIT", "rank1_dsp_split"), ("RANK1_DWC_SPLIT", "rank1_dwc_split"),
                       ("LSTM_SKIP_DPRE", "lstm_skip_dpre"), ("FUSE_GATE_LSTM", "fuse_gate_lstm"), ("LSTM_H_PLANES", "lstm_h_planes"),
                       ("DEFER_WGRAD", "defer_wgrad"), ("CHANNEL_SCALES", "channel_scales"), ("HW2_SINGLE", "hw2_single"),
@@ -89,7 +90,7 @@
                  "bn_fwd_split": 0, "bn_fwd_split_operand": 0, "bn_skip_z": 0, "bn_bwd_split": 0, "bn_skip_dx": 0,
                  "conv_bn_stats": 0, "grad_merge": 0, "rank1_dsp_split": 0, "rank1_dwc_split": 0, "lstm_skip_dpre": 0, "wgrad_multi": 0,
                  "row_sparse_bwd": 0, "fan_in_rows": 0, "direct_grad": 0, "output_gate": 0, "skinny_gemm": 0, "async_dgrad": 0,
-                 "drt_fwd_batched": 0, "rank1_fused": 0}
+                 "drt_fwd_batched": 0, "rank1_fused": 0, "bn_bwd_fold": 0, "bn_res_direct": 0}
 
 
 def _grad_slot(param):
@@ -378,7 +379,7 @@
     return flops * (1 / 1.1e14 - 1 / (4.0e14 if f16 else 2.5e14)) > split_bytes / 4e12 and flops > (1e9 if free_a else 2e9)
 
 
-def _igemm_b3(d: ConvDesc, Xs, Ws, bias, out, stats=None, rows=None):
+def _igemm_b3(d: ConvDesc, Xs, Ws, bias, out, stats=None, rows=None, bnbwd=None):
     assert Xs.scheme == Ws.scheme, (Xs.scheme, Ws.scheme)
     f16 = Xs.scheme == "f16x2"
     xscale = Xs.scale
@@ -398,6 +399,9 @@
         if stats is not None:
             check(hip.lib().sp_conv_igemm_f16x2_stats(C.byref(d), ptr(Xs.buf), ptr(xscale), ptr(Ws.buf), ptr(Ws.scale), ptr(out),
                                                       ptr(stats[0]), ptr(stats[1]), hip.stream()), "sp_conv_igemm_f16x2_stats")
+        elif bnbwd is not None:
+            check(hip.lib().sp_conv_igemm_f16x2_bnbwd(C.byref(d), ptr(Xs.buf), ptr(xscale), ptr(Ws.buf), ptr(Ws.scale), ptr(out),
+                                                      C.byref(bnbwd), hip.stream()), "sp_conv_igemm_f16x2_bnbwd")
         elif f16:
             fn = hip.lib().sp_conv_igemm_f16x1 if THROUGHPUT_MODE else hip.lib().sp_conv_igemm_f16x2
             check(fn(C.byref(d), ptr(Xs.buf), ptr(xscale), ptr(Ws.buf), ptr(Ws.scale), ptr(bias), ptr(out), hip.stream()),
@@ -522,14 +526,63 @@
     return xs, stats
 
 
-def _conv_dgrad(g: ConvGeom, dy, wp, dx, *, dys=None, wcache=None, channel=False, free_a=False, a_elems=None, beta=0, rows=None):
+class BnFoldRecord:
+    __slots__ = ("x", "mask", "mean", "invstd", "result")
+
+    def __init__(self, x, mask, mean, invstd):
+        self.x, self.mask, self.mean, self.invstd, self.result = x, mask, mean, invstd, None
+
+
+def bn_fold_fits(M: int, C_: int) -> bool:
+    return BN_BWD_FOLD and BN_SPLIT and not THROUGHPUT_MODE and M > 0 and M % 256 == 0 and C_ % 128 == 0
+
+
+def _bn_fold_args(g: ConvGeom, dx, rec, lazy):
+    if rec is None and lazy is None:
+        return None
+    M = g.N * g.H * g.W
+    ok = bn_fold_fits(M, g.Ci) and _scheme_for(g.Co) == "f16x2" and dx.data_ptr() % 16 == 0
+    if rec is not None and not (ok and rec.x is not None and rec.x.numel() == M * g.Ci and rec.x.is_contiguous() and rec.x.data_ptr() % 16 == 0):
+        rec = None
+    if lazy is not None and not (ok and lazy[0].numel() == M * g.Ci and lazy[0].is_contiguous() and lazy[0].data_ptr() % 16 == 0):
+        raise RuntimeError("scanpaths_amd: a BatchNorm left its residual gradient to this conv's data gradient (bn_bwd_fold) but the "
+                           "launch does not qualify; run with SP_BN_BWD_FOLD=0")
+    if rec is None and lazy is None:
+        return None
+    f = BnFold()
+    dep = None
+    if rec is not None:
+        G = M // 256
+        dep = (torch.empty((G, 2, g.Ci), dtype=torch.float64, device=dx.device),
+               torch.empty((G, g.Ci), dtype=torch.float32, device=dx.device), G)
+        f.x, f.mask, f.mean, f.invstd = rec.x.data_ptr(), ptr(rec.mask), rec.mean.data_ptr(), rec.invstd.data_ptr()
+        f.partial, f.dmax = dep[0].data_ptr(), dep[1].data_ptr()
+    if lazy is not None:
+        f.res_dy, f.res_mask = lazy[0].data_ptr(), ptr(lazy[1])
+    return f, dep
+
+
+def _conv_dgrad(g: ConvGeom, dy, wp, dx, *, dys=None, wcache=None, channel=False, free_a=False, a_elems=None, beta=0, rows=None,
+                fold=None, lazy=None):
     if not g.dgrad_split(free_a, a_elems):
+        if lazy is not None:
+            raise RuntimeError("scanpaths_amd: a BatchNorm left its residual gradient to this conv's data gradient (bn_bwd_fold) but "
+                               "that runs on the fp32 kernel; run with SP_BN_BWD_FOLD=0")
         _fp32_required(dy, "the fp32 data-gradient GEMM")
         _igemm(g.dgrad_desc(False, beta=beta), dy, wp, None, dx)
         return None
     if dys is None or dys.scheme != _scheme_for(g.Co):
         dys = split_op(dy, channel=channel)
-    _igemm_b3(g.dgrad_desc(True, beta=beta), dys, _weight_operand(wp, dys, wcache, transposed=True), None, dx, rows=rows)
+    args = _bn_fold_args(g, dx, fold, lazy) if (rows is None and dys.scheme == "f16x2") else None
+    if args is None and lazy is not None:
+        raise RuntimeError("scanpaths_amd: a BatchNorm left its residual gradient to this conv's data gradient (bn_bwd_fold) but the "
+                           "launch does not qualify; run with SP_BN_BWD_FOLD=0")
+    _igemm_b3(g.dgrad_desc(True, beta=beta), dys, _weight_operand(wp, dys, wcache, transposed=True), None, dx, rows=rows,
+              bnbwd=args[0] if args is not None else None)
+    if args is not None and args[1] is not None:
+        fold.result = args[1] + (dx, dx._version)
+    if lazy is not None:
+        FUSION_COUNTS["bn_res_direct"] += 1
     return dys
 
 
@@ -698,10 +751,11 @@
 
 
 class GradMerge:
-    __slots__ = ("first", "merged")
+    __slots__ = ("first", "merged", "lazy_ok", "lazy")
 
     def __init__(self):
         self.first, self.merged = None, False
+        self.lazy_ok, self.lazy = False, None
 
 
 class _Tap(Function):
@@ -714,6 +768,10 @@
     def backward(ctx, g_main, g_side):
         h = ctx.holder
         merged, h.first, h.merged = h.merged, None, False
+        if h.lazy is not None:
+            h.lazy = None
+            raise RuntimeError("scanpaths_amd: a residual gradient left for conv1's data gradient (bn_bwd_fold) was never added; run "
+                               "with SP_BN_BWD_FOLD=0")
         if g_main is None or g_side is None:
             return (g_main if g_side is None else g_side), None
         if merged:
@@ -723,7 +781,7 @@
 
 def tap(x: torch.Tensor, holder: GradMerge):
     outs = _Tap.apply(x, holder)
-    for attr in ("_sp_cache", "_sp_amax"):
+    for attr in ("_sp_cache", "_sp_amax", "_sp_bnfold"):
         v = getattr(x, attr, None)
         if v is not None:
             for o in outs:
@@ -767,6 +825,7 @@
         defer = wcache.get("defer") if isinstance(wcache, dict) else None
         ctx.defer_final = defer.claim() if (defer is not None and ctx.needs_input_grad[1]) else False
         ctx.dy_token = None
+        ctx.fold = getattr(x, "_sp_bnfold", None) if (BN_BWD_FOLD and x.is_contiguous() and grad_store is None) else None
         x = x.contiguous()
         wp = _phys(w.detach())
         assert wp.shape[3] == x.shape[3], (wp.shape, x.shape)
@@ -793,6 +852,9 @@
         xs_buf, xs_scale = (xs.buf, xs.scale) if xs is not None else (None, None)
         ctx.geom, ctx.cfg = g, (relu, bias is not None)
         ctx.wcache = wcache
+        if grad_accum is not None:
+            grad_accum.lazy_ok = bool(need_dx and bn_fold_fits(g.N * g.H * g.W, g.Ci) and _scheme_for(g.Co) == "f16x2"
+                                      and g.dgrad_split(free_a=False, a_elems=y.numel()) and step is None)
         ctx.save_for_backward(x, wp, y if relu else None, xs_buf, xs_scale)
         return y
 
@@ -810,7 +872,8 @@
             check(hip.lib().sp_relu_bwd(ptr(dy), ptr(y), dy.numel(), ptr(dyr), hip.stream()), "sp_relu_bwd")
             dy = dyr
         dx, dw = _conv_backward(ctx.geom, x, wp, dy, xs, ctx.wcache, ctx.needs_input_grad[0], ctx.needs_input_grad[1],
-                                accum=ctx.grad_accum, defer_final=ctx.defer_final, step=ctx.step, w_param=ctx.w_param)
+                                accum=ctx.grad_accum, defer_final=ctx.defer_final, step=ctx.step, w_param=ctx.w_param,
+                                fold=ctx.fold if (BN_BWD_FOLD and ctx.grad_store is None) else None)
         if ctx.grad_store is not None and dx is not None:
             ctx.grad_store.first = dx
         db = _colsum_any(dy, wp.shape[0]) if (has_bias and ctx.needs_input_grad[2]) else None
@@ -865,7 +928,8 @@
     return dwp.permute(0, 3, 1, 2)
 
 
-def _conv_backward(g: ConvGeom, x, wp, dy, xs, wcache, need_dx, need_dw, accum=None, defer_final=False, step=None, w_param=None):
+def _conv_backward(g: ConvGeom, x, wp, dy, xs, wcache, need_dx, need_dw, accum=None, defer_final=False, step=None, w_param=None,
+                   fold=None):
     dx = dw = None
     dys = None
     dy_cached = getattr(dy, "_sp_cache", None)
@@ -881,13 +945,19 @@
             deferred = True
     if need_dx:
         beta = 0
-        if accum is not None and accum.first is not None and accum.first.shape == x.shape and accum.first.is_contiguous():
+        lazy = None
+        if accum is not None and accum.lazy is not None:
+            lazy, accum.lazy, accum.merged = accum.lazy, None, True
+            dx = torch.empty_like(x)
+        elif accum is not None and accum.first is not None and accum.first.shape == x.shape and accum.first.is_contiguous():
             dx, beta, accum.merged = accum.first, 1, True
             FUSION_COUNTS["grad_merge"] += 1
         else:
             dx = torch.empty_like(x)
+        if accum is not None and not accum.merged:
+            fold = None
         dys = _conv_dgrad(g, dy, wp, dx, dys=dys, wcache=wcache, channel=True, free_a=dy_cached is not None or dys is not None,
-                          a_elems=dy.numel(), beta=beta, rows=(rc, step) if rc is not None else None) or dys
+                          a_elems=dy.numel(), beta=beta, rows=(rc, step) if rc is not None else None, fold=fold, lazy=lazy) or dys
     slot = None
     if need_dw and not deferred:
         if defer is None:
@@ -1151,6 +1221,7 @@
             y._sp_uninit = True
         ctx.cfg = (relu, residual is not None, bool(emit_bwd) and Cc % 16 == 0)
         ctx.save_for_backward(x, mask, mean, invstd, gamma.detach(), ext)
+        ctx.fold = y._sp_bnfold = BnFoldRecord(x, mask, mean, invstd) if bn_fold_fits(M, Cc) else None
         return y
 
     @staticmethod
@@ -1163,7 +1234,19 @@
         L = hip.lib()
         dev = x.device
         dx = torch.empty_like(x)
-        dres = torch.empty_like(x) if has_res else None
+        lazy_res = (has_res and BN_BWD_FOLD and ctx.res_store is not None and ctx.res_store.lazy_ok and dy.shape == x.shape
+                    and dy.data_ptr() % 16 == 0)
+        dres = torch.empty_like(x) if (has_res and not lazy_res) else None
+        pre, rec = None, ctx.fold
+        if rec is not None and rec.result is not None:
+            partial, dmax, G, gt, ver = rec.result
+            rec.result = None
+            if BN_BWD_FOLD and gt.data_ptr() == dy.data_ptr() and gt.shape == dy.shape and dy._version == ver and dy.is_contiguous():
+                pre = (partial, dmax, G)
+                FUSION_COUNTS["bn_bwd_fold"] += 1
+            del gt
+        if rec is not None:
+            rec.x = rec.mask = rec.mean = rec.invstd = None
         gslot, dgamma = _take_grad_view(ctx.params[0]) if ctx.needs_input_grad[1] else (None, None)
         bslot, dbeta = _take_grad_view(ctx.params[1]) if ctx.needs_input_grad[2] else (None, None)
         if dgamma is None:
@@ -1183,11 +1266,14 @@
         check(L.sp_bn_bwd_split(ptr(dy), ptr(x), ptr(mask), ptr(mean), ptr(invstd), ptr(gamma), ptr(ext), M, Cc,
                                 None if skip else ptr(dx),
                                 ptr(dres), ptr(planes), ptr(dhint), _hint_ptr(bhint), ptr(dgamma), ptr(dbeta), ptr(ws),
+                                ptr(pre[0]) if pre else None, ptr(pre[1]) if pre else None, pre[2] if pre else 0,
                                 hip.stream()), "sp_bn_bwd_split")
         dx._sp_amax = dhint
         if planes is not None:
             dx._sp_cache = {"f16x2": SplitOperand(planes, dhint, "f16x2")}
-        if ctx.res_store is not None and dres is not None:
+        if lazy_res:
+            ctx.res_store.lazy = (dy, mask)
+        elif ctx.res_store is not None and dres is not None:
             ctx.res_store.first = dres
         if gslot is not None:
             gslot.done()
diff --git a/scanpaths_amd/hip.py b/scanpaths_amd/hip.py
--- a/scanpaths_amd/hip.py
+++ b/scanpaths_amd/hip.py
@@ -41,6 +41,11 @@
                 ("ldo", C.c_int), ("beta", C.c_int), ("alpha", C.c_float), ("nbatch", C.c_int),
                 ("strideX", C.c_int64), ("strideY", C.c_int64), ("strideO", C.c_int64),
                 ("x_scale_vec", C.c_int), ("y_scale_vec", C.c_int), ("row_last", C.c_void_p), ("row_step", C.c_int)]
+
+
+class BnFold(C.Structure):
+    _fields_ = [("x", C.c_void_p), ("mask", C.c_void_p), ("mean", C.c_void_p), ("invstd", C.c_void_p), ("partial", C.c_void_p),
+                ("dmax", C.c_void_p), ("res_dy", C.c_void_p), ("res_mask", C.c_void_p)]
 
 
 _P, _I, _L, _F = C.c_void_p, C.c_int, C.c_int64, C.c_float
@@ -89,7 +94,8 @@
     "sp_bn_fwd_split": (_I, [_P, _L, _I, _F, _F, _P, _P, _P, _P, _I, _P, _P, _P, _P, _P, _P, _P, _P, _P, _P, _P, _P, _P, _I, _P]),
     "sp_conv_stats_tiles": (_L, [C.POINTER(ConvDesc)]),
     "sp_conv_igemm_f16x2_stats": (_I, [C.POINTER(ConvDesc), _P, _P, _P, _P, _P, _P, _P, _P]),
-    "sp_bn_bwd_split": (_I, [_P, _P, _P, _P, _P, _P, _P, _L, _I, _P, _P, _P, _P, _P, _P, _P, _P, _P]),
+    "sp_conv_igemm_f16x2_bnbwd": (_I, [C.POINTER(ConvDesc), _P, _P, _P, _P, _P, C.POINTER(BnFold), _P]),
+    "sp_bn_bwd_split": (_I, [_P, _P, _P, _P, _P, _P, _P, _L, _I, _P, _P, _P, _P, _P, _P, _P, _P, _P, _P, _I, _P]),
     "sp_sum_n": (_I, [_P, _I, _L, _P, _P, _P, _P, _I, _P]),
     "sp_sum_n_mixed": (_I, [_P, _P, _P, _I, _L, _P, _P, _P, _P, _I, _P]),
     "sp_relu_bwd": (_I, [_P, _P, _L, _P, _P]),
diff --git a/scanpaths_amd/models/scanpath_model.py b/scanpaths_amd/models/scanpath_model.py
--- a/scanpaths_amd/models/scanpath_model.py
+++ b/scanpaths_amd/models/scanpath_model.py
@@ -228,6 +228,7 @@
         if self._bn_seen:
             torch._foreach_add_(self._bn_seen, 1)
         self._bn_seen = []
+        x._sp_bnfold = None
         return x
 
     @staticmethod
```

After: 138.1 images/s (median of 4 runs). About the same (+0.3%).
